# Sorax5/RaytracingEngine

Hardware: AMD Instinct MI355X
Metric: Mrays/sec (primary+shadow) at 1920x1080 (higher is better)
Workload: dtype f64

## Files before the change

include/rt_capi.h:

```cpp
#ifndef RT_CAPI_H
#define RT_CAPI_H

#include <stddef.h>
#include <stdint.h>

#ifdef __cplusplus
extern "C" {
#endif

#define RT_CAPI_VERSION 1

typedef enum rt_status {
    RT_OK = 0,
    RT_ERR_INVALID_ARG = 1,
    RT_ERR_HIP = 2,
    RT_ERR_OOM = 3,
    RT_ERR_UNSUPPORTED = 4,
    RT_ERR_NO_DEVICE = 5,
    RT_ERR_RCCL = 6
} rt_status;

typedef struct rt_material {
    double color[3];
    double shininess;
// ... 265 lines not shown
#define RT_SC_REFRACT  0x02
#define RT_SC_REFLECT  0x04
#define RT_SC_WEIGHTS  0x08
#define RT_SC_FLAGS    0x10
#define RT_SC_ALL      0x1f
struct rt_scatter_out {
    void* value;
    void* refract_rays;
    void* reflect_rays;
    void* weights;
    void* flags;
};
rt_status rt_scatter_rays(rt_context* ctx, const rt_scene* scene, const rt_render_opts* opts,
                          const double* rays, size_t n, int outputs,
                          const struct rt_scatter_out* out);
rt_status rt_scatter_rays_device(rt_context* ctx, const rt_scene* scene,
                                 const rt_render_opts* opts, const void* d_rays, size_t n,
                                 int outputs, const struct rt_scatter_out* d_out);

rt_status rt_camera_rays(rt_context* ctx, const rt_camera* cam, const rt_render_opts* opts,
                         int sample, double* rays_out);
rt_status rt_camera_rays_device(rt_context* ctx, const rt_camera* cam, const rt_render_opts* opts,
                                int sample, void* d_rays);

#define RT_CH_T        0x01
#define RT_CH_PRIM     0x02
#define RT_CH_NORMAL   0x04
#define RT_CH_POINT    0x08
#define RT_CH_MATERIAL 0x10
#define RT_CH_ALL      0x1f
struct rt_closest_out {
    void* t;
    void* prim;
    void* normal;
    void* point;
    void* material;
};
rt_status rt_closest_rays(rt_context* ctx, const rt_scene* scene, const rt_render_opts* opts,
                          const double* rays, size_t n, int outputs,
                          const struct rt_closest_out* out);
rt_status rt_closest_rays_device(rt_context* ctx, const rt_scene* scene,
                                 const rt_render_opts* opts, const void* d_rays, size_t n,
                                 int outputs, const struct rt_closest_out* d_out);

rt_status rt_trace_rays_device(rt_context* ctx, const rt_scene* scene, const rt_render_opts* opts,
                               const void* d_rays, size_t n, void* d_rgb);

rt_status rt_accumulate_samples_device(rt_context* ctx, const rt_scene* scene,
                                       const rt_camera* cam, const rt_render_opts* opts,
                                       int sample_begin, int sample_end, void* d_sum);
rt_status rt_accumulate_samples(rt_context* ctx, const rt_scene* scene, const rt_camera* cam,
                                const rt_render_opts* opts, int sample_begin, int sample_end,
                                double* sum);

rt_status rt_resolve_device(rt_context* ctx, const void* d_sum, size_t n_pixels, int samples,
                            int tonemap, void* d_hdr64, void* d_hdr32, void* d_ldr);
rt_status rt_resolve(rt_context* ctx, const double* sum, size_t n_pixels, int samples, int tonemap,
                     double* hdr64, float* hdr32, uint8_t* ldr);

rt_status rt_tonemap(rt_context* ctx, const double* hdr, size_t n_pixels, int op,
                     uint8_t* ldr_out);

rt_status rt_debug_f64_ops(rt_context* ctx, const double* x, const double* y, size_t n,
                           double* out);

rt_status rt_debug_vec_ops(rt_context* ctx, const double* v, size_t n, double* out);

rt_status rt_debug_assemble_rows(rt_context* ctx, const void* gathered, size_t row_bytes,
                                 uint32_t height, uint32_t block, uint32_t n, uint32_t max_rows,
                                 void* image);

rt_status rt_debug_tile_order(rt_context* ctx, const rt_scene* scene, const rt_camera* cam,
                              uint32_t* order, uint32_t* cost, size_t capacity, uint32_t* tiles,
                              uint32_t* waves, int* state);

rt_status rt_debug_cone_table(rt_context* ctx, uint64_t* with_table, uint64_t* without_table);

rt_status rt_debug_shadow_table(rt_context* ctx, uint64_t* with_table, uint64_t* without_table);

rt_status rt_debug_tile_class(rt_context* ctx, uint64_t* with_words, uint64_t* without_words);

rt_status rt_debug_plane_clear(rt_context* ctx, uint64_t* with_masks, uint64_t* without_masks);

#ifdef __cplusplus
}
#endif

#endif
```

raytracingengine_amd/capi.py:

```python
from __future__ import annotations

import ctypes
import os

import numpy as np

from .scene import AREA_LIGHT_DTYPE, SceneData

HERE = os.path.dirname(os.path.abspath(__file__))
LIB_PATH = os.environ.get("RTAMD_LIB", os.path.join(HERE, "librtamd.so"))

(RT_OK, RT_ERR_INVALID_ARG, RT_ERR_HIP, RT_ERR_OOM, RT_ERR_UNSUPPORTED, RT_ERR_NO_DEVICE,
 RT_ERR_RCCL) = range(7)
STATUS_NAMES = {0: "RT_OK", 1: "RT_ERR_INVALID_ARG", 2: "RT_ERR_HIP", 3: "RT_ERR_OOM",
                4: "RT_ERR_UNSUPPORTED", 5: "RT_ERR_NO_DEVICE", 6: "RT_ERR_RCCL"}

TONEMAP_NONE = -1
TONEMAPS = ["simple", "reinhard_simple", "reinhard_extended", "reinhard_extended_luminance",
            "reinhard_jodie", "uncharted2", "aces"]
TONEMAP_ALL = 7
RT_FLAG_COUNT_RAYS = 0x1
RT_FLAG_TIME_KERNEL = 0x2
RT_FLAG_GENERIC_KERNEL = 0x4
RT_FLAG_NO_BVH = 0x8
RT_FLAG_PIPELINE = 0x10
RT_FLAG_NO_TILE_ORDER = 0x20
RT_FLAG_NO_SAMPLE_PARALLEL = 0x40
RT_OUT_HDR64, RT_OUT_HDR32, RT_OUT_LDR = 0x1, 0x2, 0x4
RT_COMM_ID_BYTES = 128
GB_DEPTH = 0x01
GB_DEPTH_NORM = 0x02
GB_NORMAL = 0x04
GB_PRIM = 0x08
GB_ALBEDO = 0x10
GB_ALL = 0x1F
DL_RADIANCE = 0x1
DL_DIFFUSE = 0x2
DL_SPECULAR = 0x4
DL_ALL = 0x7
DL_OUTPUTS = [("radiance", DL_RADIANCE), ("diffuse", DL_DIFFUSE), ("specular", DL_SPECULAR)]
SC_VALUE = 0x01
SC_REFRACT = 0x02
SC_REFLECT = 0x04
SC_WEIGHTS = 0x08
SC_FLAGS = 0x10
SC_ALL = 0x1F
SC_OUTPUTS = [("value", SC_VALUE, np.float64, 3), ("refract_rays", SC_REFRACT, np.float64, 6),
              ("reflect_rays", SC_REFLECT, np.float64, 6), ("weights", SC_WEIGHTS, np.float64, 2),
              ("flags", SC_FLAGS, np.uint8, 0)]
CH_T = 0x01
CH_PRIM = 0x02
CH_NORMAL = 0x04
CH_POINT = 0x08
CH_MATERIAL = 0x10
CH_ALL = 0x1F
CH_OUTPUTS = [("t", CH_T, np.float64, 0), ("prim", CH_PRIM, np.int32, 2),
              ("normal", CH_NORMAL, np.float64, 3), ("point", CH_POINT, np.float64, 3),
              ("material", CH_MATERIAL, np.float64, 7)]
GB_OUTPUTS = [("depth", GB_DEPTH, np.float64, 1), ("depth_norm", GB_DEPTH_NORM, np.float32, 1),
              ("normal", GB_NORMAL, np.float64, 3), ("prim", GB_PRIM, np.int32, 2),
              ("albedo", GB_ALBEDO, np.float32, 3)]

EXPORTED = [
    "rt_last_error", "rt_build_info", "rt_device_count", "rt_render_opts_default", "rt_context_create",
    "rt_context_destroy", "rt_context_set_stream", "rt_context_synchronize", "rt_scene_create",
    "rt_scene_destroy", "rt_scene_set_area_light", "rt_render", "rt_render_device",
    "rt_render_multi", "rt_comm_unique_id", "rt_comm_create", "rt_comm_create_all",
    "rt_comm_create_local", "rt_comm_destroy", "rt_comm_info", "rt_comm_set_root_weight",
    "rt_comm_create_ex", "rt_comm_set_timeout", "rt_render_gather", "rt_render_gather_all",
    "rt_comm_timing", "rt_comm_synchronize", "rt_debug_assemble_rows", "rt_debug_tile_order",
    "rt_stats_read", "rt_stats_reset", "rt_trace_rays", "rt_intersect_rays", "rt_tonemap",
    "rt_debug_f64_ops", "rt_debug_vec_ops", "rt_queue_create", "rt_queue_destroy",
    "rt_queue_submit", "rt_queue_wait", "rt_queue_synchronize", "rt_render_batch",
    "rt_render_gather_batch", "rt_render_gather_all_batch", "rt_gbuffer", "rt_gbuffer_device",
    "rt_debug_cone_table",
    "rt_debug_shadow_table",
    "rt_debug_tile_class",
    "rt_debug_plane_clear",
    "rt_occluded_rays", "rt_occluded_rays_device",
    "rt_transmittance_rays", "rt_transmittance_rays_device",
    "rt_light_transmittance", "rt_light_transmittance_device",
    "rt_direct_light", "rt_direct_light_device",
    "rt_direct_light_rays", "rt_direct_light_rays_device",
    "rt_scatter_rays", "rt_scatter_rays_device",
    "rt_camera_rays", "rt_camera_rays_device",
    "rt_closest_rays", "rt_closest_rays_device",
    "rt_trace_rays_device",
    "rt_accumulate_samples", "rt_accumulate_samples_device",
    "rt_resolve", "rt_resolve_device",
]


class RtError(RuntimeError):
    def __init__(self, status: int, msg: str):
        super().__init__(f"{STATUS_NAMES.get(status, status)}: {msg}")
        self.status = status


class SceneDesc(ctypes.Structure):
    _fields_ = [
        ("spheres", ctypes.c_void_p), ("n_spheres", ctypes.c_int32),
        ("planes", ctypes.c_void_p), ("n_planes", ctypes.c_int32),
        ("triangles", ctypes.c_void_p), ("n_triangles", ctypes.c_int32),
        ("lights", ctypes.c_void_p), ("n_lights", ctypes.c_int32),
    ]


class RenderOpts(ctypes.Structure):
    _fields_ = [
        ("max_recursion", ctypes.c_int32), ("tonemap", ctypes.c_int32),
        ("bias", ctypes.c_double), ("seed", ctypes.c_uint64),
        ("row_begin", ctypes.c_uint32), ("row_end", ctypes.c_uint32),
        ("flags", ctypes.c_int32), ("row_block", ctypes.c_uint16), ("row_cycle", ctypes.c_uint16),
    ]


class Stats(ctypes.Structure):
    _fields_ = [
        ("trace_rays", ctypes.c_uint64), ("shadow_rays", ctypes.c_uint64),
        ("kernel_ms", ctypes.c_double), ("launches", ctypes.c_uint64),
    ]


class GBufferPtrs(ctypes.Structure):
    _fields_ = [(name, ctypes.c_void_p) for name, _, _, _ in GB_OUTPUTS]


def gbuffer_layout(outputs: int, width: int, rows: int, frames: int | None = None) -> dict:
    if outputs == 0 or outputs & ~GB_ALL:
        raise ValueError(f"G-buffer outputs {outputs:#x}: no output or an unknown bit")
    lead = () if frames is None else (int(frames),)
    return {name: (lead + (rows, width) + ((k,) if k > 1 else ()), np.dtype(dt))
            for name, bit, dt, k in GB_OUTPUTS if outputs & bit}


class DirectLightPtrs(ctypes.Structure):
    _fields_ = [(name, ctypes.c_void_p) for name, _ in DL_OUTPUTS]


def material_rows(materials, n: int) -> np.ndarray:
    if hasattr(materials, "as_tuple"):
        c, *rest = materials.as_tuple()
        materials = (*c, *rest)
    m = np.ascontiguousarray(materials, np.float64)
    if m.ndim == 1:
        m = m.reshape(1, -1)
    if m.ndim != 2 or m.shape[1] != 7 or m.shape[0] not in (1, n):
        raise ValueError("materials: a Material, seven values, or an [n, 7] array")
    return m


class ScatterPtrs(ctypes.Structure):
    _fields_ = [(name, ctypes.c_void_p) for name, *_ in SC_OUTPUTS]


def _sc_check(outputs: int):
    if outputs == 0 or outputs & ~SC_ALL:
        raise ValueError("outputs: a non-empty combination of SC_* bits")


class ClosestPtrs(ctypes.Structure):
# ... 29 lines not shown
        import torch
    except ImportError:
        pass
    if not os.path.exists(path):
        raise RuntimeError(
            f"{path} is missing: build it with `python -c 'import __graft_entry__ as g; g.build()'`"
            " (hipcc --offload-arch=gfx950). The renderer has no CPU fallback.")
    L = ctypes.CDLL(path)
    vp, i32 = ctypes.c_void_p, ctypes.c_int
    L.rt_last_error.restype = ctypes.c_char_p
    if hasattr(L, "rt_build_info") or "RTAMD_LIB" not in os.environ:
        L.rt_build_info.restype = ctypes.c_char_p
        L.rt_build_info.argtypes = []
    L.rt_device_count.restype = i32
    L.rt_render_opts_default.argtypes = [vp]
    L.rt_render_opts_default.restype = None
    for name, args in {
        "rt_context_create": [i32, vp],
        "rt_context_destroy": [vp],
        "rt_context_set_stream": [vp, vp],
        "rt_context_synchronize": [vp],
        "rt_scene_create": [vp, vp, vp],
        "rt_scene_destroy": [vp],
        "rt_scene_set_area_light": [vp, vp],
        "rt_render": [vp, vp, vp, vp, vp, vp, vp, vp],
        "rt_render_device": [vp, vp, vp, vp, vp, vp, vp],
        "rt_render_batch": [vp, vp, vp, i32, vp, vp, vp, vp],
        "rt_gbuffer": [vp, vp, vp, vp, i32, vp],
        "rt_gbuffer_device": [vp, vp, vp, i32, vp, i32, vp],
        "rt_render_multi": [vp, vp, i32, vp, vp, vp, vp, vp, vp],
        "rt_stats_read": [vp, vp],
        "rt_stats_reset": [vp],
        "rt_trace_rays": [vp, vp, vp, vp, ctypes.c_size_t, vp, vp],
        "rt_intersect_rays": [vp, vp, vp, ctypes.c_size_t, vp],
        "rt_occluded_rays": [vp, vp, vp, vp, vp, ctypes.c_size_t, vp],
        "rt_occluded_rays_device": [vp, vp, vp, vp, vp, ctypes.c_size_t, vp],
        "rt_transmittance_rays": [vp, vp, vp, vp, vp, ctypes.c_size_t, vp],
        "rt_transmittance_rays_device": [vp, vp, vp, vp, vp, ctypes.c_size_t, vp],
        "rt_light_transmittance": [vp, vp, vp, vp, ctypes.c_size_t, vp],
        "rt_light_transmittance_device": [vp, vp, vp, vp, ctypes.c_size_t, vp],
        "rt_direct_light": [vp, vp, vp, vp, vp, ctypes.c_size_t, ctypes.c_size_t, i32, vp],
        "rt_direct_light_device": [vp, vp, vp, vp, vp, ctypes.c_size_t, ctypes.c_size_t, i32, vp],
        "rt_direct_light_rays": [vp, vp, vp, vp, ctypes.c_size_t, i32, vp],
        "rt_direct_light_rays_device": [vp, vp, vp, vp, ctypes.c_size_t, i32, vp],
        "rt_scatter_rays": [vp, vp, vp, vp, ctypes.c_size_t, i32, vp],
        "rt_scatter_rays_device": [vp, vp, vp, vp, ctypes.c_size_t, i32, vp],
        "rt_camera_rays": [vp, vp, vp, i32, vp],
        "rt_camera_rays_device": [vp, vp, vp, i32, vp],
        "rt_closest_rays": [vp, vp, vp, vp, ctypes.c_size_t, i32, vp],
        "rt_closest_rays_device": [vp, vp, vp, vp, ctypes.c_size_t, i32, vp],
        "rt_trace_rays_device": [vp, vp, vp, vp, ctypes.c_size_t, vp],
        "rt_accumulate_samples": [vp, vp, vp, vp, i32, i32, vp],
        "rt_accumulate_samples_device": [vp, vp, vp, vp, i32, i32, vp],
        "rt_resolve": [vp, vp, ctypes.c_size_t, i32, i32, vp, vp, vp],
        "rt_resolve_device": [vp, vp, ctypes.c_size_t, i32, i32, vp, vp, vp],
        "rt_tonemap": [vp, vp, ctypes.c_size_t, i32, vp],
        "rt_debug_f64_ops": [vp, vp, vp, ctypes.c_size_t, vp],
        "rt_debug_vec_ops": [vp, vp, ctypes.c_size_t, vp],
        "rt_comm_unique_id": [vp],
        "rt_comm_create": [vp, i32, i32, vp, vp],
        "rt_comm_create_ex": [vp, i32, i32, vp, ctypes.c_long, vp],
        "rt_comm_set_timeout": [vp, ctypes.c_long],
        "rt_comm_create_all": [vp, i32, vp],
        "rt_comm_create_local": [vp, i32, vp],
        "rt_comm_destroy": [vp],
        "rt_comm_info": [vp, vp, vp],
        "rt_comm_set_root_weight": [vp, i32],
        "rt_render_gather": [vp, vp, vp, vp, i32, vp, vp, vp],
        "rt_render_gather_all": [vp, vp, i32, vp, vp, i32, vp, vp, vp],
        "rt_render_gather_batch": [vp, vp, vp, i32, vp, i32, vp, vp, vp, vp, vp, vp],
        "rt_render_gather_all_batch": [vp, vp, i32, vp, i32, vp, i32, vp, vp, vp],
        "rt_comm_timing": [vp, vp, i32],
        "rt_comm_synchronize": [vp],
        "rt_queue_create": [vp, i32, vp],
        "rt_queue_destroy": [vp],
        "rt_queue_submit": [vp, vp, vp, vp, vp, vp, vp, vp],
        "rt_queue_wait": [vp, ctypes.c_uint64],
        "rt_queue_synchronize": [vp],
        "rt_debug_tile_order": [vp, vp, vp, vp, vp, ctypes.c_size_t, vp, vp, vp],
        "rt_debug_cone_table": [vp, vp, vp],
        "rt_debug_shadow_table": [vp, vp, vp],
        "rt_debug_tile_class": [vp, vp, vp],
        "rt_debug_plane_clear": [vp, vp, vp],
        "rt_debug_assemble_rows": [vp, vp, ctypes.c_size_t, ctypes.c_uint32, ctypes.c_uint32,
                                   ctypes.c_uint32, ctypes.c_uint32, vp],
    }.items():
        try:
            fn = getattr(L, name)
        except AttributeError:
            if "RTAMD_LIB" in os.environ:
                continue
            raise
        fn.argtypes = args
        fn.restype = i32
    _lib = L
    return L


def build_info() -> dict:
    import json
    info = json.loads(load_library().rt_build_info().decode())
    from . import build
    info["matches_tree"] = info.get("source_sha256") == build.source_digest()
    return info


def _check(status: int):
    if status != RT_OK:
        raise RtError(status, _lib.rt_last_error().decode(errors="replace"))


def rendered_rows(o: RenderOpts, height: int) -> int:
    r1 = min(o.row_end, height) if o.row_end else height
    if r1 <= o.row_begin:
        return 0
    if o.row_cycle <= 1 or o.row_block == 0:
        return r1 - o.row_begin
    stride = o.row_block * o.row_cycle
    return sum(min(o.row_block, r1 - b) for b in range(o.row_begin, r1, stride))


def default_opts(**kw) -> RenderOpts:
    o = RenderOpts()
    load_library().rt_render_opts_default(ctypes.byref(o))
    for k, v in kw.items():
        setattr(o, k, v)
    return o


def device_count() -> int:
    return load_library().rt_device_count()


def progressive_schedule(aa_samples: int) -> list:
    n = max(1, int(aa_samples))
    steps, k = [], 1
    while k < n:
        steps.append(k)
        k *= 2
    return steps + [n]


class Context:

    def __init__(self, device: int = 0):
        L = load_library()
        self._h = ctypes.c_void_p()
        _check(L.rt_context_create(device, ctypes.byref(self._h)))
        self.device = device

    def close(self):
        if self._h:
            _lib.rt_context_destroy(self._h)
            self._h = ctypes.c_void_p()

    def __del__(self):
        try:
            self.close()
        except Exception:
            pass

    def __enter__(self):
        return self

    def __exit__(self, *exc):
        self.close()

    @property
    def handle(self):
        return self._h

    def set_stream(self, stream_ptr: int | None):
        _check(_lib.rt_context_set_stream(self._h, stream_ptr))

    def synchronize(self):
        _check(_lib.rt_context_synchronize(self._h))

    def scene(self, sc: SceneData) -> "DeviceScene":
        return DeviceScene(self, sc)

    def stats(self) -> Stats:
        s = Stats()
        _check(_lib.rt_stats_read(self._h, ctypes.byref(s)))
        return s

    def reset_stats(self):
        _check(_lib.rt_stats_reset(self._h))

    def tonemap(self, hdr: np.ndarray, op: int) -> np.ndarray:
        hdr = np.ascontiguousarray(hdr, np.float64).reshape(-1, 3)
        planes = 7 if op == TONEMAP_ALL else 1
        out = np.empty((planes, hdr.shape[0], 3), np.uint8)
        _check(_lib.rt_tonemap(self._h, hdr.ctypes.data, hdr.shape[0], op, out.ctypes.data))
        return out if planes > 1 else out[0]

    def debug_f64_ops(self, x: np.ndarray, y: np.ndarray) -> np.ndarray:
        x = np.ascontiguousarray(x, np.float64)
        y = np.ascontiguousarray(y, np.float64)
        out = np.empty((x.size, 5), np.float64)
        _check(_lib.rt_debug_f64_ops(self._h, x.ctypes.data, y.ctypes.data, x.size,
                                     out.ctypes.data))
        return out

    def debug_assemble_rows(self, gathered: np.ndarray, height: int, block: int, n: int,
                            max_rows: int) -> np.ndarray:
        g = np.ascontiguousarray(gathered, np.uint8).reshape(n, max_rows, -1)
        out = np.empty((height, g.shape[2]), np.uint8)
        _check(_lib.rt_debug_assemble_rows(self._h, g.ctypes.data, g.shape[2], height, block, n,
                                           max_rows, out.ctypes.data))
        return out

    def debug_cone_table(self) -> tuple[int, int]:
        a, b = ctypes.c_uint64(), ctypes.c_uint64()
        _check(_lib.rt_debug_cone_table(self._h, ctypes.byref(a), ctypes.byref(b)))
        return a.value, b.value

    def debug_shadow_table(self) -> tuple[int, int]:
        a, b = ctypes.c_uint64(), ctypes.c_uint64()
        _check(_lib.rt_debug_shadow_table(self._h, ctypes.byref(a), ctypes.byref(b)))
        return a.value, b.value

    def debug_tile_class(self) -> tuple[int, int]:
        a, b = ctypes.c_uint64(), ctypes.c_uint64()
        _check(_lib.rt_debug_tile_class(self._h, ctypes.byref(a), ctypes.byref(b)))
        return a.value, b.value

    def debug_plane_clear(self) -> tuple[int, int]:
        a, b = ctypes.c_uint64(), ctypes.c_uint64()
        _check(_lib.rt_debug_plane_clear(self._h, ctypes.byref(a), ctypes.byref(b)))
        return a.value, b.value

    def debug_vec_ops(self, v: np.ndarray) -> np.ndarray:
        v = np.ascontiguousarray(v, np.float64).reshape(-1, 3)
        out = np.empty((v.shape[0], 16), np.float64)
        _check(_lib.rt_debug_vec_ops(self._h, v.ctypes.data, v.shape[0], out.ctypes.data))
        return out


class DeviceScene:

    def __init__(self, ctx: Context, sc: SceneData):
        self.ctx = ctx
        self.data = sc
        self._arrays = (sc.sphere_array(), sc.plane_array(), sc.triangle_array(), sc.light_array())
        sp, pl, tr, lt = self._arrays
        desc = SceneDesc(sp.ctypes.data if len(sp) else None, len(sp),
                         pl.ctypes.data if len(pl) else None, len(pl),
                         tr.ctypes.data if len(tr) else None, len(tr),
                         lt.ctypes.data if len(lt) else None, len(lt))
        self._h = ctypes.c_void_p()
        _check(_lib.rt_scene_create(ctx.handle, ctypes.byref(desc), ctypes.byref(self._h)))
        self.camera = sc.camera.to_struct()
        self._area = None
        if sc.area_light is not None:
            self._area = sc.area_light.to_struct()
            _check(_lib.rt_scene_set_area_light(self._h, self._area.ctypes.data))

    def close(self):
        if self._h:
            _lib.rt_scene_destroy(self._h)
            self._h = ctypes.c_void_p()

    def __del__(self):
        try:
            self.close()
        except Exception:
            pass

    def render(self, *, hdr64=True, hdr32=False, tonemap: int = TONEMAP_NONE, opts=None,
               stats=False, **opt_kw):
        cam = self.data.camera
        o = opts if opts is not None else default_opts(tonemap=tonemap, **opt_kw)
        if opts is None:
            o.tonemap = tonemap
        rows = rendered_rows(o, cam.height)
        out = {}
        a64 = np.empty((rows, cam.width, 3), np.float64) if hdr64 else None
        a32 = np.empty((rows, cam.width, 3), np.float32) if hdr32 else None
        ldr = np.empty((rows, cam.width, 3), np.uint8) if tonemap != TONEMAP_NONE else None
        st = Stats()
        _check(_lib.rt_render(self.ctx.handle, self._h, self.camera.ctypes.data, ctypes.byref(o),
                              a64.ctypes.data if a64 is not None else None,
                              a32.ctypes.data if a32 is not None else None,
                              ldr.ctypes.data if ldr is not None else None,
                              ctypes.byref(st) if stats else None))
        if a64 is not None:
            out["hdr64"] = a64
        if a32 is not None:
            out["hdr32"] = a32
        if ldr is not None:
            out["ldr"] = ldr
        if stats:
            out["trace_rays"] = st.trace_rays
            out["shadow_rays"] = st.shadow_rays
        return out

    def render_host(self, h_hdr64: int | None, h_hdr32: int | None, h_ldr: int | None,
                    opts: RenderOpts, stats: bool = False):
        st = Stats()
        _check(_lib.rt_render(self.ctx.handle, self._h, self.camera.ctypes.data, ctypes.byref(opts),
                              h_hdr64, h_hdr32, h_ldr, ctypes.byref(st) if stats else None))
        return st if stats else None

    def trace_rays(self, rays: np.ndarray, stats=False, **opt_kw):
        rays = np.ascontiguousarray(rays, np.float64).reshape(-1, 6)
        out = np.empty((rays.shape[0], 3), np.float64)
        o = default_opts(**opt_kw)
        st = Stats()
        _check(_lib.rt_trace_rays(self.ctx.handle, self._h, ctypes.byref(o), rays.ctypes.data,
                                  rays.shape[0], out.ctypes.data,
                                  ctypes.byref(st) if stats else None))
        return (out, st) if stats else out
# ... 702 lines not shown
```

raytracingengine_amd/csrc/rt_capi.cpp:

```cpp
#include "rt_capi.h"

#include <hip/hip_runtime.h>

#include <algorithm>
#include <cmath>
#include <cstdlib>
#include <cstdio>
#include <cstring>
#include <mutex>
#include <new>
#include <string>
#include <utility>
#include <vector>

#include "rt_context.hpp"
#include "rt_internal.hpp"
#include "rt_wavefront.hpp"

#pragma clang fp contract(off)

using namespace rtamd;

namespace rtamd {

// ... 202 lines not shown
        if (ctx->scratch_used) RT_HIP(hipEventSynchronize(ctx->scratch_event));
        RT_HIP(ctx->fix_list.ensure(px * sizeof(uint32_t)));
    }
    p.fix_list = static_cast<uint32_t*>(ctx->fix_list.ptr);
    p.fix_ctl = static_cast<uint32_t*>(ctx->fix_ctl.ptr) + ctx->fix_parity;
    p.fix_next = static_cast<uint32_t*>(ctx->fix_ctl.ptr) + (1 - ctx->fix_parity);
    return RT_OK;
}

rt_status check_batch(const rt_camera* cams, int nframes) {
    if (!cams || nframes < 1) return fail(RT_ERR_INVALID_ARG, "frame batch: no cameras");
    for (int f = 0; f < nframes; ++f) {
        rt_status st = validate_camera(cams + f);
        if (st != RT_OK) return st;
        if (cams[f].width != cams[0].width || cams[f].height != cams[0].height ||
            cams[f].aa_samples != cams[0].aa_samples ||
            std::memcmp(&cams[f].focal, &cams[0].focal, sizeof(double)) != 0)
            return fail(RT_ERR_INVALID_ARG, "frame batch: every camera must have the first's "
                                            "width, height, focal and aa_samples");
    }
    return RT_OK;
}

rt_status enqueue_render(rt_context* ctx, const rt_scene* sc, const rt_camera* cam,
                         const rt_render_opts* opts, double* d64, float* d32, uint8_t* dldr) {
    return enqueue_frames(ctx, sc, cam, 1, opts, d64, d32, dldr);
}

rt_status enqueue_frames(rt_context* ctx, const rt_scene* sc, const rt_camera* cams, int nframes,
                         const rt_render_opts* opts, double* d64, float* d32, uint8_t* dldr,
                         uint32_t frame_rows) {
    TraceParams p;
    int path;
    bool lds;
    size_t lds_bytes;
    uint32_t rows;
    rt_status st = nframes == 1 ? RT_OK : check_batch(cams, nframes);
    if (st != RT_OK) return st;
    st = build_params(ctx, sc, cams, opts, p, path, lds, lds_bytes, rows);
    if (st != RT_OK) return st;
    p.out64 = d64;
    p.out32 = d32;
    p.ldr = dldr;
    const int flags = opts ? opts->flags : 0;
    if (!dldr) p.tonemap = RT_TONEMAP_NONE;
    if (dldr && p.tonemap == RT_TONEMAP_NONE) p.ldr = nullptr;
    const bool packet_path = path == kPathDirect && !(flags & RT_FLAG_GENERIC_KERNEL) &&
                             p.ns <= packet_max_spheres() &&
                             packet_lds_bytes(p.ns, p.np, p.nl) <= ctx->lds_limit;
    if (frame_rows && frame_rows < rows)
        return fail(RT_ERR_INVALID_ARG, "frame batch: frame stride below the rendered rows");
    const size_t frame_px = static_cast<size_t>(frame_rows ? frame_rows : rows) * p.width;
    if (nframes > 1 && (!packet_path || nframes > kPkMaxBatch)) {
        const int step = packet_path ? kPkMaxBatch : 1;
        for (int f0 = 0; f0 < nframes; f0 += step) {
            const size_t off = 3 * frame_px * static_cast<size_t>(f0);
            st = enqueue_frames(ctx, sc, cams + f0, std::min(step, nframes - f0), opts,
                                d64 ? d64 + off : nullptr, d32 ? d32 + off : nullptr,
                                dldr ? dldr + off : nullptr, frame_rows);
            if (st != RT_OK) return st;
        }
        return RT_OK;
    }
    bool scratch = (flags & RT_FLAG_COUNT_RAYS) || uses_wavefront_arena(path, flags);

    std::pair<hipEvent_t, hipEvent_t> ev{nullptr, nullptr};
    if (flags & RT_FLAG_TIME_KERNEL) {
        if (ctx->pending.size() >= 1024) {
            st = harvest_events(ctx, false);
            if (st != RT_OK) return st;
        }
        if (!ctx->free_events.empty()) {
            ev = ctx->free_events.back();
            ctx->free_events.pop_back();
        } else {
            RT_HIP(hipEventCreate(&ev.first));
            RT_HIP(hipEventCreate(&ev.second));
        }
        RT_HIP(hipEventRecord(ev.first, ctx->stream));
    }
    const bool packet = packet_path;
    rt_scene::PkImage::TileOrder* rec = nullptr;
    int batch_ring = -1;
    if (packet && nframes > 1) {
        p.nframes = static_cast<uint32_t>(nframes);
        p.frame_px = frame_px;
        st = packet_batch_images(ctx, sc, cams, nframes, p, flags, &rec, &batch_ring);
        if (st != RT_OK) return st;
    } else if (packet) {
        st = packet_image(ctx, sc, p, flags, &rec);
        if (st != RT_OK) return st;
    }
    if (packet) {
        for (int f = 0; f < nframes; ++f)
            ++((nframes > 1 ? p.fr_tab[f] : p.cone_tab) ? ctx->cone_tab_frames
                                                         : ctx->cone_notab_frames);
        for (int f = 0; f < nframes; ++f)
            ++((nframes > 1 ? p.fr_stab[f] : p.shadow_tab) ? ctx->shadow_tab_frames
                                                            : ctx->shadow_notab_frames);
        for (int f = 0; f < nframes; ++f)
            ++((nframes > 1 ? p.fr_ctab[f] : p.class_tab) ? ctx->tile_class_frames
                                                          : ctx->tile_noclass_frames);
        for (int f = 0; f < nframes; ++f)
            ++(((nframes > 1 ? p.fr_ctab[f] : p.class_tab) && p.plane_masks)
                   ? ctx->plane_mask_frames
                   : ctx->plane_nomask_frames);
    }
    const bool fixup = packet && packet_uses_fixup(p, false, sc->max_specular > 0.0);
    if (fixup) {
        st = fixup_buffers(ctx, nframes > 1 ? static_cast<size_t>(nframes) * frame_px
                                             : static_cast<size_t>(rows) * p.width, p);
        if (st != RT_OK) return st;
        scratch = true;
    }
    if (scratch) {
        st = scratch_wait(ctx);
        if (st != RT_OK) return st;
    }
    const bool lean_generic = p.nt == 0 && p.al_samples == 0;
    static const bool box_sph = [] {
        const char* e = std::getenv("RTAMD_BOX_SPH");
        return !(e && std::atoi(e) == 0);
    }();
    const bool box = path == kPathChain && p.nt == 0 && p.al_samples == 0 &&
                     (p.ns == 0 ? p.np > 0 : (box_sph && p.ns <= kBoxMaxSpheres)) &&
                     !(flags & RT_FLAG_GENERIC_KERNEL);
    const bool spar = !(flags & RT_FLAG_NO_SAMPLE_PARALLEL);
    auto launch = [&](const TraceParams& q, bool count) {
        if (box)
            return launch_box_chain(q, count, !(flags & RT_FLAG_NO_SAMPLE_PARALLEL), ctx->stream);
        return packet ? launch_packet_direct(q, count, sc->max_specular > 0.0, ctx->stream)
                      : (lean_generic ? lean::launch_trace(q, path, count, lds, lds_bytes, ctx->stream, spar)
                                      : launch_trace(q, path, count, lds, lds_bytes, ctx->stream, spar));
    };
    bool wavefront = false;
    if (uses_wavefront_arena(path, flags)) {
        const size_t n0 = static_cast<size_t>(rows) * p.width *
                          static_cast<size_t>(p.aa > 0 ? p.aa : 0);
        const char* env = std::getenv("RTAMD_WF_MB");
        const size_t budget = (env && std::atoll(env) > 0 ? static_cast<size_t>(std::atoll(env))
                                                          : size_t(4096)) << 20;
        const bool defer = path == kPathTree && wf_defer_selected();
        const size_t root_bytes = wf_arena_bytes(n0, n0, defer);
        if (n0 < (size_t(1) << 30) && root_bytes <= budget) {
            size_t extra = (budget - root_bytes) / (defer ? 116 : 100);
            extra = std::min(extra, std::max<size_t>(n0, 1) * 64);
            extra = std::min(extra, (size_t(1) << 31) - 1 - n0);
            const size_t cap = n0 + extra;
            RT_HIP(ctx->wf.ensure(wf_arena_bytes(n0, cap, defer)));
            RT_HIP(ctx->wf_ctl.ensure(sizeof(WfCtl)));
            const WfArena A = wf_arena_layout(ctx->wf.ptr, n0, cap,
                                              static_cast<WfCtl*>(ctx->wf_ctl.ptr), defer);
            RT_HIP(lean_generic ? lean::launch_wavefront(p, path, A, lds, lds_bytes, ctx->stream)
                                : launch_wavefront(p, path, A, lds, lds_bytes, ctx->stream));
            wavefront = true;
        }
    }
    if (!wavefront) RT_HIP(launch(p, false));
    if (fixup) {
        const hipError_t fe = launch_packet_fixup(p, ctx->stream);
        if (fe != hipSuccess) {
            (void)hipMemsetAsync(ctx->fix_ctl.ptr, 0, 2 * sizeof(uint32_t), ctx->stream);
            return hip_fail(fe, "launch_packet_fixup");
        }
        ctx->fix_parity ^= 1;
    }
    if (rec) RT_HIP(hipEventRecord(rec->recorded, ctx->stream));
    if (flags & RT_FLAG_TIME_KERNEL) {
        RT_HIP(hipEventRecord(ev.second, ctx->stream));
        ctx->pending.push_back(ev);
    }
    if (flags & RT_FLAG_COUNT_RAYS) {
        TraceParams pc = p;
        pc.out64 = nullptr;
        pc.out32 = nullptr;
        pc.ldr = nullptr;
        pc.counters = static_cast<unsigned long long*>(ctx->counters.ptr);
        pc.tile_cost = nullptr;
        RT_HIP(launch(pc, true));
    }
    if (batch_ring >= 0) {
        RT_HIP(hipEventRecord(sc->pk_batch_done[batch_ring], ctx->stream));
        sc->pk_batch_used[batch_ring] = true;
    }
    return scratch ? scratch_done(ctx) : RT_OK;
}

constexpr size_t kGbBytes[5] = {8, 4, 24, 8, 12};

rt_status check_gbuffer_args(int outputs, const rt_gbuffer_out* out) {
    if (outputs == 0) return fail(RT_ERR_INVALID_ARG, "G-buffer: no output requested");
    if (outputs & ~RT_GB_ALL) return fail(RT_ERR_INVALID_ARG, "G-buffer: unknown output bit");
    if (!out) return fail(RT_ERR_INVALID_ARG, "G-buffer: the output record is NULL");
    const void* ptr[5] = {out->depth, out->depth_norm, out->normal, out->prim, out->albedo};
    for (int k = 0; k < 5; ++k)
        if ((outputs & (1 << k)) && !ptr[k])
            return fail(RT_ERR_INVALID_ARG, "G-buffer: a requested output's pointer is NULL");
    return RT_OK;
}

rt_status enqueue_gbuffer(rt_context* ctx, const rt_scene* sc, const rt_camera* cams, int nframes,
                          const rt_render_opts* opts_in, int outputs, const rt_gbuffer_out& out) {
    rt_status st = check_batch(cams, nframes);
    if (st != RT_OK) return st;
    rt_render_opts opts;
    if (opts_in) opts = *opts_in;
    else rt_render_opts_default(&opts);
    opts.max_recursion = 1;
    opts.tonemap = RT_TONEMAP_NONE;
    opts.flags &= RT_FLAG_GENERIC_KERNEL | RT_FLAG_NO_BVH | RT_FLAG_TIME_KERNEL;
    TraceParams p;
    int path;
    bool lds;
    size_t lds_bytes;
// ... 242 lines not shown
    }

    if (sc->ns >= kSphChunkMin) {
        std::vector<int32_t> perm;
        std::vector<double> bnd;
        build_sphere_chunks(&h[sc->off_sph], sc->ns, perm, bnd);
        sc->off_sbnd = (h.size() + 1) & ~size_t(1);
        sc->off_sperm = sc->off_sbnd + bnd.size();
        h.resize(sc->off_sperm + (perm.size() + 1) / 2 + 2, 0.0);
        std::memcpy(&h[sc->off_sbnd], bnd.data(), bnd.size() * sizeof(double));
        std::memcpy(&h[sc->off_sperm], perm.data(), perm.size() * sizeof(int32_t));
    }

    if (sc->np > 0) {
        std::vector<int> grp(sc->np);
        for (int i = 0; i < sc->np; ++i) {
            const double* q = &h[sc->off_pl + size_t(kPlStride) * i];
            const double* n = q + 3;
            grp[i] = 3;
            const bool bounded = std::fabs(q[0]) <= 0x1p1000 && std::fabs(q[1]) <= 0x1p1000 &&
                                 std::fabs(q[2]) <= 0x1p1000;
            for (int k = 0; k < 3 && bounded; ++k)
                if (std::fabs(n[k]) == 1.0 && n[(k + 1) % 3] == 0.0 && n[(k + 2) % 3] == 0.0)
                    grp[i] = k;
        }
        sc->off_box = (h.size() + 1) & ~size_t(1);
        h.resize(sc->off_box + size_t(kBoxRec) * sc->np + 2, 0.0);
        size_t r = 0;
        for (int g = 0; g < 4; ++g) {
            for (int i = 0; i < sc->np; ++i) {
                if (grp[i] != g) continue;
                const double* pl = &h[sc->off_pl + size_t(kPlStride) * i];
                double* o = &h[sc->off_box + size_t(kBoxRec) * r++];
                for (int k = 0; k < 6; ++k) o[k] = pl[k];
                o[6] = g < 3 ? pl[g] : 0.0;
                const double nn = pl[3] * pl[3] + pl[4] * pl[4] + pl[5] * pl[5];
                o[7] = std::sqrt(nn) == 1.0 ? 1.0 : 0.0;
                for (int k = 0; k < kMatStride - 1; ++k)
                    o[8 + k] = h[sc->off_pl_mat + size_t(kMatStride) * i + k];
                const int32_t idx[2] = {i, 0};
                std::memcpy(&o[15], idx, sizeof idx);
                ++sc->box_n[g];
            }
        }
    }

    hipError_t e = sc->buf.ensure(h.size() * sizeof(double));
    if (e == hipSuccess)
        e = hipMemcpyAsync(sc->buf.ptr, h.data(), h.size() * sizeof(double),
                           hipMemcpyHostToDevice, ctx->stream);
    if (e == hipSuccess) e = hipStreamSynchronize(ctx->stream);
    if (e != hipSuccess) {
        sc->buf.release();
        delete sc;
        return hip_fail(e, "rt_scene_create upload");
    }
    *out = sc;
    return RT_OK;
}

rt_status rt_scene_destroy(rt_scene* sc) {
    if (!sc) return RT_OK;
    DeviceGuard g(sc->ctx->device);
    (void)hipDeviceSynchronize();
    sc->buf.release();
    sc->pk_pub.release();
    sc->pk_batch.release();
    for (auto& e : sc->pk_batch_done)
        if (e) (void)hipEventDestroy(e);
    for (auto& im : sc->pk_images) {
        im.buf.release();
        if (im.ready) (void)hipEventDestroy(im.ready);
        for (auto& o : im.ords) {
            o.cost.release();
            o.keys.release();
            o.order.release();
            if (o.recorded) (void)hipEventDestroy(o.recorded);
            if (o.built) (void)hipEventDestroy(o.built);
            if (o.verdict) (void)hipHostFree(o.verdict);
        }
        for (auto& t : im.tabs) {
            t.buf.release();
            if (t.ready) (void)hipEventDestroy(t.ready);
        }
    }
    for (auto& b : sc->pk_batch_tab) b.release();
    delete sc;
    return RT_OK;
}

rt_status rt_scene_set_area_light(rt_scene* sc, const rt_area_light* light) {
    if (!sc) return fail(RT_ERR_INVALID_ARG, "scene is NULL");
    if (!light) {
        sc->has_area = false;
        return RT_OK;
    }
    if (light->samples <= 0) return fail(RT_ERR_INVALID_ARG, "area light needs samples > 0");
    const int k = static_cast<int>(std::lround(std::sqrt(static_cast<double>(light->samples))));
    if (k * k != light->samples)
        return fail(RT_ERR_INVALID_ARG, "area light samples must be a perfect square");
    sc->area = *light;
    sc->has_area = true;
    return RT_OK;
}

rt_status rt_render_device(rt_context* ctx, const rt_scene* sc, const rt_camera* cam,
                           const rt_render_opts* opts, void* d64, void* d32, void* dldr) {
    if (!ctx) return fail(RT_ERR_INVALID_ARG, "context is NULL");
    DeviceGuard g(ctx->device);
    return enqueue_render(ctx, sc, cam, opts, static_cast<double*>(d64), static_cast<float*>(d32),
                   static_cast<uint8_t*>(dldr));
}

rt_status rt_render_batch(rt_context* ctx, const rt_scene* sc, const rt_camera* cams,
                          int nframes, const rt_render_opts* opts, void* d64, void* d32,
                          void* dldr) {
    if (!ctx) return fail(RT_ERR_INVALID_ARG, "context is NULL");
    rt_status st = check_batch(cams, nframes);
    if (st != RT_OK) return st;
    DeviceGuard g(ctx->device);
    return enqueue_frames(ctx, sc, cams, nframes, opts, static_cast<double*>(d64),
                          static_cast<float*>(d32), static_cast<uint8_t*>(dldr));
}

rt_status rt_gbuffer_device(rt_context* ctx, const rt_scene* sc, const rt_camera* cams,
                            int nframes, const rt_render_opts* opts, int outputs,
                            const struct rt_gbuffer* d_out) {
    rt_status st = check_gbuffer_args(outputs, d_out);
    if (st != RT_OK) return st;
    if (!ctx) return fail(RT_ERR_INVALID_ARG, "context is NULL");
    DeviceGuard g(ctx->device);
    return enqueue_gbuffer(ctx, sc, cams, nframes, opts, outputs, *d_out);
}

rt_status rt_gbuffer(rt_context* ctx, const rt_scene* sc, const rt_camera* cam,
                     const rt_render_opts* opts, int outputs, const struct rt_gbuffer* h_out) {
    rt_status st = check_gbuffer_args(outputs, h_out);
    if (st != RT_OK) return st;
    if (!ctx) return fail(RT_ERR_INVALID_ARG, "context is NULL");
    st = validate_camera(cam);
    if (st != RT_OK) return st;
    DeviceGuard g(ctx->device);
    rt_render_opts o;
    if (opts) o = *opts;
    else rt_render_opts_default(&o);
    const size_t npx = static_cast<size_t>(rendered_rows(o, cam->height)) * cam->width;
    void* const host[5] = {h_out->depth, h_out->depth_norm, h_out->normal, h_out->prim,
                           h_out->albedo};
    size_t off[5], total = 0;
    for (int k = 0; k < 5; ++k) {
        off[k] = total;
        if (outputs & (1 << k)) total += (npx * kGbBytes[k] + 255) / 256 * 256;
    }
    RT_HIP(ctx->out64.ensure(total));
    char* base = static_cast<char*>(ctx->out64.ptr);
    rt_gbuffer_out d{base + off[0], base + off[1], base + off[2], base + off[3], base + off[4]};
    st = enqueue_gbuffer(ctx, sc, cam, 1, &o, outputs, d);
    if (st != RT_OK) return st;
    for (int k = 0; k < 5; ++k)
        if (outputs & (1 << k))
            RT_HIP(hipMemcpyAsync(host[k], base + off[k], npx * kGbBytes[k], hipMemcpyDeviceToHost,
                                  ctx->stream));
    RT_HIP(hipStreamSynchronize(ctx->stream));
    return RT_OK;
}

// ... 863 lines not shown
    return RT_OK;
}

rt_status rt_debug_f64_ops(rt_context* ctx, const double* x, const double* y, size_t n,
                           double* out) {
    if (!ctx || !x || !y || !out) return fail(RT_ERR_INVALID_ARG, "NULL argument");
    DeviceGuard g(ctx->device);
    RT_HIP(ctx->dbg.ensure(n * 7 * sizeof(double)));
    double* dx = static_cast<double*>(ctx->dbg.ptr);
    double* dy = dx + n;
    double* dout = dy + n;
    RT_HIP(hipMemcpyAsync(dx, x, n * sizeof(double), hipMemcpyHostToDevice, ctx->stream));
    RT_HIP(hipMemcpyAsync(dy, y, n * sizeof(double), hipMemcpyHostToDevice, ctx->stream));
    RT_HIP(launch_debug_f64(dx, dy, n, dout, ctx->stream));
    RT_HIP(hipMemcpyAsync(out, dout, 5 * n * sizeof(double), hipMemcpyDeviceToHost, ctx->stream));
    RT_HIP(hipStreamSynchronize(ctx->stream));
    return RT_OK;
}

rt_status rt_debug_tile_order(rt_context* ctx, const rt_scene* sc, const rt_camera* cam,
                              uint32_t* order, uint32_t* cost, size_t capacity, uint32_t* tiles,
                              uint32_t* waves, int* state) {
    if (!ctx || !sc || !cam || !tiles || !waves || !state)
        return fail(RT_ERR_INVALID_ARG, "NULL argument to rt_debug_tile_order");
    *tiles = *waves = 0;
    *state = 0;
    DeviceGuard g(ctx->device);
    RT_HIP(hipDeviceSynchronize());
    for (const auto& im : sc->pk_images) {
        if (std::memcmp(im.cam, cam->position, sizeof im.cam) != 0) continue;
        if (im.last_ord < 0) return RT_OK;
        const auto& o = im.ords[static_cast<size_t>(im.last_ord)];
        *state = o.state;
        if (o.state == 0) return RT_OK;
        *tiles = o.key[0] * o.key[1];
        *waves = o.key[2];
        if (order && o.state == 2) {
            if (capacity < *tiles) return fail(RT_ERR_INVALID_ARG, "order capacity too small");
            RT_HIP(hipMemcpy(order, o.order.ptr, sizeof(uint32_t) * *tiles, hipMemcpyDeviceToHost));
        }
        if (cost) {
            if (capacity < size_t(*tiles) * *waves)
                return fail(RT_ERR_INVALID_ARG, "cost capacity too small");
            RT_HIP(hipMemcpy(cost, o.cost.ptr, sizeof(uint32_t) * *tiles * *waves,
                             hipMemcpyDeviceToHost));
        }
        return RT_OK;
    }
    return RT_OK;
}

rt_status rt_debug_cone_table(rt_context* ctx, uint64_t* with_table, uint64_t* without_table) {
    if (!ctx || !with_table || !without_table)
        return fail(RT_ERR_INVALID_ARG, "NULL argument to rt_debug_cone_table");
    *with_table = ctx->cone_tab_frames;
    *without_table = ctx->cone_notab_frames;
    return RT_OK;
}

rt_status rt_debug_shadow_table(rt_context* ctx, uint64_t* with_table, uint64_t* without_table) {
    if (!ctx || !with_table || !without_table)
        return fail(RT_ERR_INVALID_ARG, "NULL argument to rt_debug_shadow_table");
    *with_table = ctx->shadow_tab_frames;
    *without_table = ctx->shadow_notab_frames;
    return RT_OK;
}

rt_status rt_debug_tile_class(rt_context* ctx, uint64_t* with_words, uint64_t* without_words) {
    if (!ctx || !with_words || !without_words)
        return fail(RT_ERR_INVALID_ARG, "NULL argument to rt_debug_tile_class");
    *with_words = ctx->tile_class_frames;
    *without_words = ctx->tile_noclass_frames;
    return RT_OK;
}

rt_status rt_debug_plane_clear(rt_context* ctx, uint64_t* with_masks, uint64_t* without_masks) {
    if (!ctx || !with_masks || !without_masks)
        return fail(RT_ERR_INVALID_ARG, "NULL argument to rt_debug_plane_clear");
    *with_masks = ctx->plane_mask_frames;
    *without_masks = ctx->plane_nomask_frames;
    return RT_OK;
}

rt_status rt_debug_vec_ops(rt_context* ctx, const double* v, size_t n, double* out) {
    if (!ctx || !v || !out) return fail(RT_ERR_INVALID_ARG, "NULL argument");
    DeviceGuard g(ctx->device);
    RT_HIP(ctx->dbg.ensure(n * 19 * sizeof(double)));
    double* dv = static_cast<double*>(ctx->dbg.ptr);
    double* dout = dv + 3 * n;
    RT_HIP(hipMemcpyAsync(dv, v, 3 * n * sizeof(double), hipMemcpyHostToDevice, ctx->stream));
    RT_HIP(launch_debug_vec(dv, n, dout, ctx->stream));
    RT_HIP(hipMemcpyAsync(out, dout, 16 * n * sizeof(double), hipMemcpyDeviceToHost, ctx->stream));
    RT_HIP(hipStreamSynchronize(ctx->stream));
    return RT_OK;
}

}
```

raytracingengine_amd/csrc/rt_context.hpp:

```cpp
#pragma once

#include <hip/hip_runtime.h>

#include <array>
#include <string>
#include <utility>
#include <vector>

#include "rt_capi.h"
#include "rt_internal.hpp"

namespace rtamd {

rt_status fail(rt_status st, const std::string& msg);
rt_status hip_fail(hipError_t e, const char* what);

#define RT_HIP(call)                                    \
    do {                                                \
        hipError_t e_ = (call);                         \
        if (e_ != hipSuccess) return rtamd::hip_fail(e_, #call); \
    } while (0)

struct DeviceBuffer {
    void* ptr = nullptr;
    size_t bytes = 0;
    hipError_t ensure(size_t need) {
        if (need <= bytes) return hipSuccess;
        if (ptr) (void)hipFree(ptr);
        ptr = nullptr;
        bytes = 0;
        hipError_t e = hipMalloc(&ptr, need);
        if (e == hipSuccess) bytes = need;
        return e;
    }
    void release() {
        if (ptr) (void)hipFree(ptr);
        ptr = nullptr;
        bytes = 0;
    }
};

struct DeviceGuard {
    int prev = -1;
    explicit DeviceGuard(int dev) {
        if (hipGetDevice(&prev) != hipSuccess) prev = -1;
        (void)hipSetDevice(dev);
    }
    ~DeviceGuard() {
        if (prev >= 0) (void)hipSetDevice(prev);
    }
};

}

struct rt_comm;

struct rt_context {
    int device = 0;
    hipStream_t stream = nullptr;
    hipStream_t own_stream = nullptr;
    size_t lds_limit = 0;
    rtamd::DeviceBuffer out64, out32, ldr, tm_in, tm_out, dbg, rays;
    rtamd::DeviceBuffer counters;
    rtamd::DeviceBuffer wf, wf_ctl;
    hipEvent_t scratch_event = nullptr;
    bool scratch_used = false;
    hipStream_t scratch_stream = nullptr;
    rtamd::DeviceBuffer fix_list, fix_ctl;
    int fix_parity = 0;
    std::vector<std::pair<hipEvent_t, hipEvent_t>> pending;
    std::vector<std::pair<hipEvent_t, hipEvent_t>> free_events;
    double timed_ms = 0.0;
    uint64_t launches = 0;
    uint64_t cone_tab_frames = 0, cone_notab_frames = 0;
    uint64_t shadow_tab_frames = 0, shadow_notab_frames = 0;
    uint64_t tile_class_frames = 0, tile_noclass_frames = 0;
    uint64_t plane_mask_frames = 0, plane_nomask_frames = 0;
    std::vector<rt_context*> group_ctxs;
    std::vector<rt_comm*> group_comms;
    std::vector<rt_context*> group_roots;
};

struct rt_scene {
    rt_context* ctx = nullptr;
    rtamd::DeviceBuffer buf;
    int32_t ns = 0, np = 0, nt = 0, nl = 0;
    size_t off_sph = 0, off_sph_mat = 0, off_pl = 0, off_pl_mat = 0, off_tri = 0, off_tri_mat = 0,
           off_lt = 0;
    bool any_transparent = false;
    double max_specular = 0.0;
    bool has_area = false;
    rt_area_light area{};
    size_t off_bvh = 0, off_bvh_tri = 0;
    int32_t bvh_nodes = 0;
    size_t off_sperm = 0, off_sbnd = 0;
    size_t off_box = 0;
    int32_t box_n[4] = {0, 0, 0, 0};
    struct PkImage {
        double cam[3];
        rtamd::DeviceBuffer buf;
        hipEvent_t ready = nullptr;
        hipStream_t stream = nullptr;
        bool done = false;
        struct TileOrder {
            uint32_t key[8] = {};
            int state = 0;
            rtamd::DeviceBuffer cost, keys, order;
            hipEvent_t recorded = nullptr, built = nullptr;
            uint32_t* verdict = nullptr;
        };
        std::vector<TileOrder> ords;
        int last_ord = -1;
        struct ConeTab {
            static constexpr size_t kKeyWords = 20;
            uint32_t key[kKeyWords] = {};
            rtamd::DeviceBuffer buf;
            hipEvent_t ready = nullptr;
            hipStream_t stream = nullptr;
            bool done = false;
        };
        std::vector<ConeTab> tabs;
    };
    mutable std::vector<PkImage> pk_images;
    mutable std::vector<std::array<double, 3>> pk_seen;
    mutable rtamd::DeviceBuffer pk_pub;
    static constexpr int kPkBatchRing = 4;
    mutable rtamd::DeviceBuffer pk_batch;
    mutable hipEvent_t pk_batch_done[kPkBatchRing] = {nullptr, nullptr, nullptr, nullptr};
    mutable bool pk_batch_used[kPkBatchRing] = {false, false, false, false};
    mutable int pk_batch_next = 0;
    mutable rtamd::DeviceBuffer pk_batch_tab[kPkBatchRing];
};

namespace rtamd {

uint32_t rendered_rows(const rt_render_opts& o, uint32_t height);
rt_status validate_camera(const rt_camera* cam);
rt_status enqueue_render(rt_context* ctx, const rt_scene* sc, const rt_camera* cam,
                         const rt_render_opts* opts, double* d64, float* d32, uint8_t* dldr);
rt_status enqueue_frames(rt_context* ctx, const rt_scene* sc, const rt_camera* cams, int nframes,
                         const rt_render_opts* opts, double* d64, float* d32, uint8_t* dldr,
                         uint32_t frame_rows = 0);
rt_status check_batch(const rt_camera* cams, int nframes);
rt_status packet_image(rt_context* ctx, const rt_scene* sc, TraceParams& p, int flags,
                       rt_scene::PkImage::TileOrder** rec);
rt_status packet_batch_images(rt_context* ctx, const rt_scene* sc, const rt_camera* cams,
                              int nframes, TraceParams& p, int flags,
                              rt_scene::PkImage::TileOrder** rec, int* batch_ring);
bool uses_wavefront_arena(int path, int flags);
rt_status scratch_wait(rt_context* ctx);
rt_status scratch_done(rt_context* ctx);
rt_status harvest_events(rt_context* ctx, bool all);
void release_group(rt_context* ctx);
void leave_groups(rt_context* ctx);

}
```

raytracingengine_amd/csrc/rt_internal.hpp:

```cpp
#pragma once

#include <hip/hip_runtime.h>
#include <stddef.h>
#include <stdint.h>

#include <vector>

namespace rtamd {

constexpr int kSphStride = 4;
constexpr int kPlStride = 8;
constexpr int kTriStride = 12;
constexpr int kLtStride = 8;
constexpr int kMatStride = 8;
constexpr int kBoxRec = 16;
constexpr int kBoxMaxSpheres = 64;

constexpr int kBvhNodeStride = 8;
constexpr int kBvhMinTris = 32;
constexpr int kBvhStack = 64;
constexpr int kMaxDepth = 16;
constexpr int kTileW = 8;
constexpr int kTileH = 32;

enum PathKind : int {
    kPathDirect = 0,
    kPathChain = 1,
    kPathTree = 2
};

constexpr int kPkMaxBatch = 32;
struct PkFrame {
    double cam[3];
    const double* img;
    unsigned long long* pub;
    uint32_t epoch;
    uint32_t _pad;
};

struct TraceParams {
    const double* sph;
    const double* sph_mat;
    const double* pl;
    const double* pl_mat;
    const double* tri;
    const double* tri_mat;
    const double* lt;
    int32_t ns, np, nt, nl;
    double al_corner[3];
    double al_u[3];
    double al_v[3];
    double al_E[3];
    int32_t al_samples;
    int32_t al_k;
    double cam_pos[3];
    double focal;
    uint32_t width, height;
    int32_t aa;
    int32_t max_rec;
    double bias;
    uint64_t seed;
    uint32_t row0, rows;
    uint32_t row_block, row_stride;
    double* out64;
    float* out32;
    uint8_t* ldr;
    int32_t tonemap;
    int32_t _pad;
    unsigned long long* counters;
    const uint8_t* redo;
    const double* bvh;
    const int32_t* bvh_tri;
    const double* pk_image;
    unsigned long long* pk_pub;
    uint32_t pk_epoch;
    uint32_t pk_pub_first;
    const int32_t* sph_perm;
    const double* sph_bnd;
    const uint32_t* redo_any;
    const uint32_t* tile_order;
    uint32_t* tile_cost;
    const double* box;
    int32_t box_n[4];
    uint32_t* fix_list;
    uint32_t* fix_ctl;
    uint32_t* fix_next;
    uint32_t nframes;
    uint32_t plane_masks;
    uint64_t frame_px;
    PkFrame fr[kPkMaxBatch];
    double half_w, half_h, cam_dz, cam_dz2;
    double fr_dz[kPkMaxBatch][2];
    const unsigned long long* cone_tab;
    const unsigned long long* fr_tab[kPkMaxBatch];
    const unsigned long long* shadow_tab;
    const unsigned long long* fr_stab[kPkMaxBatch];
    const unsigned long long* class_tab;
    const unsigned long long* fr_ctab[kPkMaxBatch];
};
static_assert(sizeof(TraceParams) + 12 * kPkMaxBatch + 32 <= 4096, "kernel arguments above 4 KiB");

struct CameraConsts {
    double half_w, half_h, dz, dz2;
};
inline CameraConsts camera_consts(uint32_t width, uint32_t height, double cam_z, double focal) {
    CameraConsts c;
    c.half_w = static_cast<double>(width) / 2.0;
    c.half_h = static_cast<double>(height) / 2.0;
    c.dz = (cam_z + focal) - cam_z;
    c.dz2 = c.dz * c.dz;
    return c;
}

constexpr int kSphChunkMin = 65;
void build_sphere_chunks(const double* sph, int ns, std::vector<int32_t>& perm,
                         std::vector<double>& bounds);

void build_triangle_bvh(const double* tri, int nt, std::vector<double>& nodes,
                        std::vector<int32_t>& order);

__host__ __device__ inline size_t scene_doubles(const TraceParams& p) {
    return static_cast<size_t>(kSphStride) * p.ns + static_cast<size_t>(kPlStride) * p.np +
           static_cast<size_t>(kLtStride) * p.nl;
}

constexpr int kAaParallelMax = 128;
hipError_t launch_trace(const TraceParams& p, int path, bool count, bool lds, size_t lds_bytes,
                        hipStream_t stream, bool sample_parallel = false);
namespace lean {
hipError_t launch_trace(const TraceParams& p, int path, bool count, bool lds, size_t lds_bytes,
                        hipStream_t stream, bool sample_parallel = false);
}
hipError_t launch_box_chain(const TraceParams& p, bool count, bool sample_parallel,
                            hipStream_t stream);
hipError_t launch_packet_direct(const TraceParams& p, bool count, bool any_specular,
                                hipStream_t stream);
size_t packet_lds_bytes(int ns, int np, int nl);
hipError_t launch_packet_image(const TraceParams& p, double* img, hipStream_t stream);
bool packet_uses_fixup(const TraceParams& p, bool count, bool any_specular);
hipError_t launch_packet_fixup(const TraceParams& p, hipStream_t stream);
struct PkImageJobs {
    double* dst[kPkMaxBatch];
    int32_t frame[kPkMaxBatch];
    int32_t n;
};
hipError_t launch_packet_image_batch(const TraceParams& p, const PkImageJobs& jobs,
                                     hipStream_t stream);
struct PkConeJobs {
    unsigned long long* dst[kPkMaxBatch];
    int32_t frame[kPkMaxBatch];
    int32_t n;
    int32_t shadow_nl;
    int32_t class_words;
};
hipError_t launch_packet_cone_tables(const TraceParams& p, const PkConeJobs& jobs,
                                     hipStream_t stream);
bool packet_reads_cone_table(const TraceParams& p, bool any_specular);
int packet_shadow_table_lights(const TraceParams& p);
void packet_grid(const TraceParams& p, uint32_t& gx, uint32_t& gy, uint32_t& waves);
hipError_t launch_packet_order(const uint32_t* cost, uint32_t gx, uint32_t gy, uint32_t waves,
                               uint32_t* keys, uint32_t* order, uint32_t* verdict,
                               hipStream_t stream);
int packet_max_spheres();
struct GbOut {
    double* depth;
    float* depth_norm;
    double* normal;
    int32_t* prim;
    float* albedo;
    double planes[kPkMaxBatch][2];
};
bool gbuffer_packet_fits(const TraceParams& p, size_t lds_limit);
hipError_t launch_gbuffer(const TraceParams& p, const GbOut& g, bool packet, int tile_w,
                          hipStream_t stream);
hipError_t launch_trace_rays(const TraceParams& p, int path, bool count, const double* rays,
                             size_t n, double* out, hipStream_t stream);
hipError_t launch_intersect_rays(const TraceParams& p, const double* rays, size_t n, double* out,
                                 hipStream_t stream);
hipError_t launch_occluded_rays(const TraceParams& p, const double* rays, const double* max_dist,
                                size_t n, uint8_t* out, hipStream_t stream);
hipError_t launch_transmittance_rays(const TraceParams& p, bool opaque, const double* rays,
                                     const double* max_dist, size_t n, double* out,
                                     hipStream_t stream);
hipError_t launch_light_transmittance(const TraceParams& p, bool opaque, const double* points,
                                      size_t n, double* out, hipStream_t stream);
struct DlOut {
    double* radiance;
    double* diffuse;
    double* specular;
};
struct DlMaterial {
    double v[8];
};
hipError_t launch_direct_light_points(const TraceParams& p, bool opaque, const double* points,
                                      const double* materials, const DlMaterial& shared, size_t n,
                                      const DlOut& out, hipStream_t stream);
hipError_t launch_direct_light_rays(const TraceParams& p, bool opaque, const double* rays, size_t n,
                                    const DlOut& out, hipStream_t stream);
struct ScOut {
    double* value;
    double* refract_rays;
    double* reflect_rays;
    double* weights;
    uint8_t* flags;
};
hipError_t launch_scatter_rays(const TraceParams& p, bool opaque, const double* rays, size_t n,
                               const ScOut& out, hipStream_t stream);
hipError_t launch_camera_rays(const TraceParams& p, int sample, double* out, hipStream_t stream);
struct ChOut {
    double* t;
    int32_t* prim;
    double* normal;
    double* point;
    double* material;
};
hipError_t launch_closest_rays(const TraceParams& p, const double* rays, size_t n, const ChOut& out,
                               hipStream_t stream);
hipError_t launch_accumulate_samples(const TraceParams& p, int path, int s0, int s1, double* sum,
                                     hipStream_t stream);
hipError_t launch_resolve(const double* sum, size_t n, int samples, int op, double* out64,
                          float* out32, uint8_t* ldr, hipStream_t stream);
hipError_t launch_tonemap(const double* hdr, size_t n, int op, uint8_t* out, hipStream_t stream);
hipError_t launch_debug_f64(const double* x, const double* y, size_t n, double* out,
                            hipStream_t stream);
hipError_t launch_debug_vec(const double* v, size_t n, double* out, hipStream_t stream);

}
```

raytracingengine_amd/csrc/rt_packet.hip:

```cpp
#include "rt_cone_table.hpp"
#include "rt_packet_kernel.hpp"
#include "rt_shadow_table.hpp"

#pragma clang fp contract(off)

namespace rtamd {

#ifdef RT_PACKET_PROBE
template __global__ void packet_direct_kernel<RT_PACKET_PROBE>(TraceParams);
#else
size_t packet_lds_bytes(int ns, int np, int nl) { return pk_image_bytes(ns, np, nl); }

__global__ __launch_bounds__(256) void packet_image_kernel(TraceParams P, double* img) {
    pk_build_image(P, P.cam_pos, img, static_cast<int>(threadIdx.x), 256);
}

hipError_t launch_packet_image(const TraceParams& p, double* img, hipStream_t stream) {
    hipLaunchKernelGGL(packet_image_kernel, dim3(1), dim3(256), 0, stream, p, img);
    return hipGetLastError();
}

__global__ __launch_bounds__(256) void packet_image_batch_kernel(TraceParams P, PkImageJobs J) {
    const int f = J.frame[blockIdx.x];
    pk_build_image(P, P.fr[f].cam, J.dst[blockIdx.x], static_cast<int>(threadIdx.x), 256);
}

hipError_t launch_packet_image_batch(const TraceParams& p, const PkImageJobs& jobs,
                                     hipStream_t stream) {
    if (jobs.n <= 0) return hipSuccess;
    if (jobs.n > kPkMaxBatch) return hipErrorInvalidValue;
    for (int j = 0; j < jobs.n; ++j)
        if (!jobs.dst[j] || jobs.frame[j] < 0 || jobs.frame[j] >= static_cast<int>(p.nframes))
            return hipErrorInvalidValue;
    hipLaunchKernelGGL(packet_image_batch_kernel, dim3(static_cast<unsigned>(jobs.n)),
                       dim3(256), 0, stream, p, jobs);
    return hipGetLastError();
}

constexpr int kConeThreads = 256;
__global__ __launch_bounds__(kConeThreads, 5) void packet_cone_table_kernel(TraceParams P,
                                                                         PkConeJobs J, uint32_t gx,
                                                                         uint32_t gy,
                                                                         uint32_t waves) {
    __shared__ float s_terms[64 * 8];
    __shared__ double s_ctr[64 * 3];
    const int f = J.frame[blockIdx.y];
    const double* camp = f < 0 ? P.cam_pos : P.fr[f].cam;
    const double* img = f < 0 ? P.pk_image : P.fr[f].img;
    const double dz = f < 0 ? P.cam_dz : P.fr_dz[f][0];
    const int ns = P.ns < 64 ? P.ns : 64;
    for (int i = threadIdx.x; i < 8 * ns; i += kConeThreads)
        s_terms[i] = reinterpret_cast<const float*>(img + kPkSph * (i >> 3) + 4)[i & 7];
    if (J.shadow_nl > 0)
        for (int i = threadIdx.x; i < 3 * ns; i += kConeThreads)
            s_ctr[i] = img[kPkSph * (i / 3) + i % 3];
    __syncthreads();
    const uint32_t t = blockIdx.x * kConeThreads + threadIdx.x;
    if (t >= gx * gy * waves) return;
    const uint32_t wave = t % waves, wg = t / waves, tbx = wg % gx, tby = wg / gx;
    const uint32_t x0 = tbx * (kPkW * kWgWavesX) + (wave % kWgWavesX) * kPkW;
    const uint32_t yl0 = tby * (kPkH * (waves / kWgWavesX)) + (wave / kWgWavesX) * kPkH;
    const ConeRowPlan rp{P.row0, P.rows, P.row_block, P.row_stride};
    const ConeRect q = cone_tile_rect(x0, yl0, P.width, rp);
    const ConeBound B = cone_tile_bound(q, P.half_w, P.half_h, camp[0], camp[1], dz);
    const uint64_t cone = cone_tile_mask(B, s_terms, 8, ns);
    J.dst[blockIdx.y][t] = cone;
    if (J.shadow_nl <= 0) return;
    unsigned long long* sw = J.dst[blockIdx.y] + static_cast<size_t>(gx) * gy * waves +
                             static_cast<size_t>(t) * J.shadow_nl;
    ShadowBound<2> SB;
    SB.n = 0;
    SB.ok = false;
    if (cone == 0)
        SB = shadow_tile_bound<2>(q, P.half_w, P.half_h, camp, dz, img + kPkSph * ns, P.np, P.bias);
    unsigned long long any = 0, keep = 0;
    for (int l = 0; l < J.shadow_nl; ++l) {
        sw[l] = shadow_tile_word(SB, P.lt + kLtStride * l, P.bias, s_ctr, 3, s_terms + 7, 8, ns);
        any |= sw[l];
        const unsigned k = J.class_words == 2
                               ? shadow_plane_keep<2>(SB, P.lt + kLtStride * l, img + kPkSph * ns,
                                                      P.np, camp, P.bias)
                               : kPlaneKeepAll;
        keep |= static_cast<unsigned long long>(k) << (8 + 8 * l);
    }
    if (J.class_words == 0) return;
    const double* pln = img + kPkSph * ns + kPlStride * P.np + kLtStride * P.nl;
    J.dst[blockIdx.y][static_cast<size_t>(gx) * gy * waves * (1 + J.shadow_nl) + t] =
        tile_class_word(cone, SB, &any, 1, pln, P.np) | keep;
}

hipError_t launch_packet_cone_tables(const TraceParams& p, const PkConeJobs& jobs,
                                     hipStream_t stream) {
    if (jobs.n <= 0) return hipSuccess;
    if (jobs.n > kPkMaxBatch || p.ns > 64 || p.width == 0 || p.rows == 0)
        return hipErrorInvalidValue;
    if (jobs.shadow_nl != 0 && jobs.shadow_nl != packet_shadow_table_lights(p))
        return hipErrorInvalidValue;
    if (jobs.class_words != 0 && jobs.shadow_nl <= 0) return hipErrorInvalidValue;
    if (jobs.class_words < 0 || jobs.class_words > 2) return hipErrorInvalidValue;
    for (int j = 0; j < jobs.n; ++j) {
        const int f = jobs.frame[j];
        if (!jobs.dst[j] || f < -1 || f >= static_cast<int>(p.nframes) ||
            !(f < 0 ? p.pk_image : p.fr[f].img))
            return hipErrorInvalidValue;
    }
    uint32_t gx, gy, waves;
    packet_grid(p, gx, gy, waves);
    const uint32_t tiles = gx * gy * waves;
    hipLaunchKernelGGL(packet_cone_table_kernel,
                       dim3((tiles + kConeThreads - 1) / kConeThreads,
                            static_cast<unsigned>(jobs.n)),
                       dim3(kConeThreads), 0, stream, p, jobs, gx, gy, waves);
    return hipGetLastError();
}

constexpr int kFixThreads = 256;
constexpr int kFixBlocks = 256;
template <bool LDS>
__global__ __launch_bounds__(kFixThreads) void packet_fixup_kernel(TraceParams P) {
    extern __shared__ double smem[];
    const uint32_t n = *P.fix_ctl;
    if (blockIdx.x == 0 && threadIdx.x == 0) *P.fix_next = 0u;
    if (blockIdx.x * kFixThreads >= n) return;
    SceneView S = stage_scene<LDS>(P, smem, threadIdx.x, kFixThreads);
    S.nt = 0;
    S.al = 0;
    S.spec = false;
    S.tri = S.tri_mat = S.bvh = nullptr;
    S.bvh_tri = nullptr;
    Counts cnt{0u, 0u};
    const uint32_t fpx = P.nframes ? static_cast<uint32_t>(P.frame_px) : 0u;
    for (uint32_t i = blockIdx.x * kFixThreads + threadIdx.x; i < n; i += gridDim.x * kFixThreads) {
        const uint32_t o = P.fix_list[i];
        const uint32_t z = fpx ? o / fpx : 0u;
        const uint32_t pl = o - z * fpx;
        const uint32_t yl = pl / P.width;
        const uint32_t x = pl - yl * P.width;
        const double* cp = P.nframes ? P.fr[z].cam : P.cam_pos;
        const d3 cam = mk(cp[0], cp[1], cp[2]);
        const uint32_t y = image_row(P, yl);
        const uint64_t pix = static_cast<uint64_t>(y) * P.width + x;
        const d3 d = camera_dir(P, cam, x, y, pix, 0);
        d3 acc = mk(0.0, 0.0, 0.0);
        acc = acc + trace_direct<false>(S, P, cam, d, pix, 0u, cnt);
        store_pixel(P, static_cast<size_t>(o), acc);
    }
}

hipError_t launch_packet_fixup(const TraceParams& p, hipStream_t stream) {
    if (!p.fix_list || !p.fix_ctl || !p.fix_next) return hipErrorInvalidValue;
    if (p.nt != 0 || p.al_samples != 0) return hipErrorInvalidValue;
    const size_t lds = sizeof(double) * scene_doubles(p);
    if (lds <= 32 * 1024)
        hipLaunchKernelGGL(packet_fixup_kernel<true>, dim3(kFixBlocks), dim3(kFixThreads), lds,
                           stream, p);
    else
        hipLaunchKernelGGL(packet_fixup_kernel<false>, dim3(kFixBlocks), dim3(kFixThreads), 0,
                           stream, p);
    return hipGetLastError();
}

int packet_max_spheres() { return 16 * 64; }

void packet_grid(const TraceParams& p, uint32_t& gx, uint32_t& gy, uint32_t& waves) {
    const size_t lds = pk_image_bytes(p.ns, p.np, p.nl);
    const uint32_t wgy = pk_wgy(lds);
    gx = (p.width + kPkW * kWgWavesX - 1) / (kPkW * kWgWavesX);
    gy = (p.rows + kPkH * wgy - 1) / (kPkH * wgy);
    waves = kWgWavesX * wgy;
}

constexpr int kOrderBins = 16;
__global__ __launch_bounds__(1024) void packet_order_kernel(const uint32_t* cost, uint32_t gx,
                                                            uint32_t gy, uint32_t waves,
                                                            uint32_t* keys, uint32_t* order,
                                                            uint32_t* verdict) {
    __shared__ uint32_t s_max, s_cnt[kOrderBins];
    const uint32_t tid = threadIdx.x, tiles = gx * gy;
    if (tid == 0) s_max = 0;
    if (tid < kOrderBins) s_cnt[tid] = 0;
    __syncthreads();
    uint32_t m = 0;
    for (uint32_t i = tid; i < tiles; i += blockDim.x) {
        uint32_t c = 0;
        for (uint32_t w = 0; w < waves; ++w) c = max(c, cost[i * waves + w]);
        keys[i] = c;
        m = max(m, c);
    }
    atomicMax(&s_max, m);
    __syncthreads();
    const uint64_t top = static_cast<uint64_t>(s_max) + 1;
    for (uint32_t i = tid; i < tiles; i += blockDim.x) {
        const uint64_t bin = static_cast<uint64_t>(keys[i]) * kOrderBins / top;
        const uint32_t key = kOrderBins - 1 - static_cast<uint32_t>(bin);
        keys[i] = key;
// ... 8 lines not shown
        if (2 * acc >= tiles) {
            median_bin = kOrderBins - 1 - b;
            break;
        }
    }
    const bool narrow = median_bin >= kOrderBins / 4;
    if (tid == 0 && verdict) __hip_atomic_store(verdict, narrow ? 1u : 2u, __ATOMIC_RELAXED,
                                                __HIP_MEMORY_SCOPE_SYSTEM);
    uint32_t cur = 0;
    for (int b = 0; b < kOrderBins; ++b)
        if (static_cast<int>(tid) > b) cur += s_cnt[b];
    if (narrow) {
        for (uint32_t lin = tid; lin < tiles; lin += 64) order[lin] = (gy - 1 - lin / gx) * gx + lin % gx;
        return;
    }
    const uint64_t below = (1ull << tid) - 1ull;
    for (uint32_t c0 = 0; c0 < tiles; c0 += 64) {
        const uint32_t lin = c0 + tid;
        const bool ok = lin < tiles;
        uint32_t tile = 0, key = kOrderBins;
        if (ok) {
            tile = (gy - 1 - lin / gx) * gx + lin % gx;
            key = keys[tile];
        }
        for (int b = 0; b < kOrderBins; ++b) {
            const uint64_t mk_ = __ballot(key == static_cast<uint32_t>(b));
            if (!mk_) continue;
            const uint32_t base = __builtin_amdgcn_readlane(cur, b);
            if (key == static_cast<uint32_t>(b))
                order[base + __builtin_popcountll(mk_ & below)] = tile;
            if (static_cast<int>(tid) == b) cur += __builtin_popcountll(mk_);
        }
    }
}

hipError_t launch_packet_order(const uint32_t* cost, uint32_t gx, uint32_t gy, uint32_t waves,
                               uint32_t* keys, uint32_t* order, uint32_t* verdict,
                               hipStream_t stream) {
    hipLaunchKernelGGL(packet_order_kernel, dim3(1), dim3(1024), 0, stream, cost, gx, gy, waves,
                       keys, order, verdict);
    return hipGetLastError();
}

template <int MAXC>
static void launch_packet_maxc(const TraceParams& p, bool count, size_t lds, int feat,
                               hipStream_t stream) {
    if (feat == kFeatFix) launch_packet_variant<1, kFeatFix>(p, count, lds, stream);
    else if (feat == 0) launch_packet_variant<MAXC, 0>(p, count, lds, stream);
    else if (feat == kFeatPlanes) launch_packet_variant<MAXC, kFeatPlanes>(p, count, lds, stream);
    else if (feat == kFeatTris) launch_packet_variant<MAXC, kFeatTris>(p, count, lds, stream);
    else launch_packet_variant<MAXC, kFeatAll>(p, count, lds, stream);
}

static int packet_features(const TraceParams& p, bool any_specular) {
    int feat = 0;
    if (any_specular) feat |= kFeatSpec;
    if (p.al_samples > 0) feat |= kFeatArea;
    if (p.nt > 0) feat |= kFeatTris;
    if (p.ldr && p.tonemap == 4) feat |= kFeatJodie;
    if (p.np >= 3 && feat == 0) feat = kFeatPlanes;
    return feat;
}

bool packet_reads_cone_table(const TraceParams& p, bool any_specular) {
    return p.aa == 1 && !p.tile_cost && p.ns >= 1 && p.ns <= 64 && p.max_rec > 0 &&
           packet_features(p, any_specular) == 0;
}

int packet_shadow_table_lights(const TraceParams& p) {
    return p.np <= 2 ? shadow_table_lights(p.ns, p.np, p.nl, p.al_samples > 0) : 0;
}

constexpr uint64_t kPkFixMinPixels = 32ull << 20;
bool packet_uses_fixup(const TraceParams& p, bool count, bool any_specular) {
    const char* e = std::getenv("RTAMD_PK_FIX");
    const int mode = e ? std::atoi(e) : -1;
    if (mode == 0) return false;
    const bool eligible = !count && p.aa == 1 && !p.tile_cost && p.nframes >= 1 &&
                          (p.ns + 63) / 64 <= 1 && packet_features(p, any_specular) == 0;
    const uint64_t px = static_cast<uint64_t>(p.nframes) * p.rows * p.width;
    return eligible && (mode == 1 || px >= kPkFixMinPixels);
}

hipError_t launch_packet_direct(const TraceParams& p, bool count, bool any_specular,
                                hipStream_t stream) {
    const size_t lds = packet_lds_bytes(p.ns, p.np, p.nl);
    const int chunks = (p.ns + 63) / 64;
    int feat = packet_features(p, any_specular);
    if (packet_uses_fixup(p, count, any_specular)) {
        if (!p.fix_list || !p.fix_ctl || !p.fix_next) return hipErrorInvalidValue;
        feat = kFeatFix;
    }
    if (feat == kFeatArea) return launch_packet_area(p, count, lds, chunks, stream);
    if (chunks <= 1) launch_packet_maxc<1>(p, count, lds, feat, stream);
    else if (chunks <= 4) launch_packet_maxc<4>(p, count, lds, feat, stream);
    else launch_packet_maxc<16>(p, count, lds, feat, stream);
    return hipGetLastError();
}
#endif

}
```

raytracingengine_amd/csrc/rt_packet_device.hpp:

```cpp
#pragma once

#include <cstdlib>

#include "rt_trace_common.hpp"

#pragma clang fp contract(off)

namespace rtamd {

constexpr int kPkW = 8;
constexpr int kPkH = 8;
#ifndef RT_PK_WAVES_X
#define RT_PK_WAVES_X 2
#endif
constexpr int kWgWavesX = RT_PK_WAVES_X;
constexpr size_t kLdsPerCu = 160 * 1024;
constexpr unsigned pk_wgy(size_t lds) { return 10 * lds <= kLdsPerCu ? 1u : 2u; }
constexpr double kCullRel = 1e-4;
constexpr double kFarRatio = 1e5;
constexpr double kNoWin = 1.0 + 0x1.0p-40;
#ifndef RT_SHADOW_SPLIT
#define RT_SHADOW_SPLIT 1
#endif
#ifndef RT_SHADOW_SPLIT_MIN
#define RT_SHADOW_SPLIT_MIN 16
#endif
constexpr bool kShadowSplit = RT_SHADOW_SPLIT != 0;
constexpr int kShadowSplitMin = RT_SHADOW_SPLIT_MIN;

constexpr int kFeatSpec = 1;
constexpr int kFeatArea = 2;
constexpr int kFeatTris = 4;
constexpr int kFeatJodie = 8;
constexpr int kFeatPlanes = 16;
constexpr int kFeatAll = 31;
constexpr int kFeatNoPL = 32;
constexpr int kFeatFix = 128;
#ifndef RT_PACKET_FIX_WAVES
#define RT_PACKET_FIX_WAVES 8
#endif

constexpr int kPkStack = 64;
#ifndef RT_PACKET_SMALL_WAVES
#define RT_PACKET_SMALL_WAVES 6
#endif
#ifndef RT_PACKET_AREA_WAVES
#define RT_PACKET_AREA_WAVES 6
#endif
#ifndef RT_PACKET_LEAN_WAVES
#define RT_PACKET_LEAN_WAVES 4
#endif
#ifndef RT_PACKET_TRIS_WAVES
#define RT_PACKET_TRIS_WAVES 4
#endif
#ifndef RT_PACKET_AA1_WAVES
#define RT_PACKET_AA1_WAVES 5
#endif

__device__ __forceinline__ int cull_lane() {
    int l;
    __asm__ volatile("v_mbcnt_lo_u32_b32 %0, -1, 0\n\tv_mbcnt_hi_u32_b32 %0, -1, %0" : "=v"(l));
    return l;
}


constexpr int kPkSph = 10;

struct PacketScene {
    const double* sph;
    const double* pl;
    const double* lt;
    const double* tri;
    const double* mat;
    const double* bvh;
    const int32_t* bvh_tri;
    const int32_t* orig;
    int ns, np, nt, nl, nb;
    int* wstk;
};

struct PkHit {
    double t;
    int prim;
};

template <int MAXC>
struct Masks {
    uint64_t m[MAXC];
    uint64_t pm;
};

template <int MAXC>
__device__ __forceinline__ Masks<MAXC> all_candidates(int ns) {
    Masks<MAXC> M;
#pragma unroll
    for (int c = 0; c < MAXC; ++c) {
        const int left = ns - 64 * c;
        M.m[c] = left >= 64 ? ~0ull : (left <= 0 ? 0ull : ((1ull << left) - 1ull));
    }
    M.pm = ~0ull;
    return M;
}

constexpr float kF32Slack = 2e-5f;
constexpr float kF32Up = 1.0f + 1e-6f;

__device__ __forceinline__ float f32_up(double v) { return static_cast<float>(v) * kF32Up; }
__device__ __forceinline__ float dot3f(float ax, float ay, float az, float bx, float by, float bz) {
    return ax * bx + ay * by + az * bz;
}
__device__ __forceinline__ float sqrt_f32(float x) { return __builtin_amdgcn_sqrtf(x); }

__device__ __forceinline__ void cone_terms(const double* s, double radius, d3 o, float* out) {
    const float r = f32_up(radius);
    const float vx = static_cast<float>(s[0] - o.x), vy = static_cast<float>(s[1] - o.y),
                vz = static_cast<float>(s[2] - o.z);
    const float dv2 = dot3f(vx, vy, vz, vx, vy, vz);
    const float rr = r * (1.0f + static_cast<float>(kCullRel));
    const float dv = sqrt_f32(dv2);
    const bool always = !(dv > 1.01f * rr) || !(dv <= static_cast<float>(kFarRatio) * r);
    out[0] = vx;
    out[1] = vy;
// ... 468 lines not shown
```

raytracingengine_amd/csrc/rt_packet_host.cpp:

```cpp
#include <hip/hip_runtime.h>

#include <algorithm>
#include <array>
#include <atomic>
#include <cstdlib>
#include <cstring>

#include "rt_context.hpp"
#include "rt_internal.hpp"

#pragma clang fp contract(off)

namespace rtamd {
namespace {

constexpr size_t kMaxPkImages = 16;
constexpr size_t kMaxPkSeen = 16;
constexpr size_t kMaxTileOrders = 8;
constexpr size_t kPkPubSlots = 32;
constexpr size_t kPkPubMaxWords = 1024;
std::atomic<uint32_t> g_pk_epoch{0};
rt_status packet_publish_slot(rt_context* ctx, const rt_scene* sc, TraceParams& p) {
    const size_t words = packet_lds_bytes(p.ns, p.np, p.nl) / 4;
    static const bool off = [] {
        const char* e = std::getenv("RTAMD_PK_PUB");
        return e && std::atoi(e) == 0;
    }();
    if (off || words > kPkPubMaxWords) return RT_OK;
    const size_t slot = kPkPubMaxWords * sizeof(unsigned long long);
    if (!sc->pk_pub.ptr) {
        RT_HIP(sc->pk_pub.ensure(kPkPubSlots * slot));
        RT_HIP(hipMemsetAsync(sc->pk_pub.ptr, 0, kPkPubSlots * slot, ctx->stream));
        RT_HIP(hipStreamSynchronize(ctx->stream));
    }
    uint32_t ep = ++g_pk_epoch;
    if (ep == 0) ep = ++g_pk_epoch;
    p.pk_epoch = ep;
    static const long first_env = [] {
        const char* e = std::getenv("RTAMD_PK_PUB_FIRST");
        return e ? std::atol(e) : -1L;
    }();
    int cus = 0;
    RT_HIP(hipDeviceGetAttribute(&cus, hipDeviceAttributeMultiprocessorCount, ctx->device));
    p.pk_pub_first = first_env >= 0 ? static_cast<uint32_t>(first_env)
                                    : static_cast<uint32_t>(cus > 0 ? cus : 256) * 10u;
    p.pk_pub = reinterpret_cast<unsigned long long*>(static_cast<char*>(sc->pk_pub.ptr) +
                                                     (ep % kPkPubSlots) * slot);
    return RT_OK;
}
rt_status tile_order(rt_context* ctx, rt_scene::PkImage& im, TraceParams& p, int flags,
                     rt_scene::PkImage::TileOrder** rec, bool existing_only = false) {
    *rec = nullptr;
    if (flags & RT_FLAG_NO_TILE_ORDER) return RT_OK;
    uint32_t gx, gy, waves;
    packet_grid(p, gx, gy, waves);
    const uint32_t key[8] = {gx, gy, waves, p.width, p.height, p.rows, p.row0,
                             (p.row_block << 16) ^ p.row_stride};
    const uint32_t tiles = gx * gy;
    size_t idx = 0;
    while (idx < im.ords.size() && std::memcmp(im.ords[idx].key, key, sizeof key) != 0) ++idx;
    if (existing_only && (idx == im.ords.size() || im.ords[idx].state != 2)) return RT_OK;
    if (idx == im.ords.size()) {
        if (im.ords.size() >= kMaxTileOrders) return RT_OK;
        if (im.ords.capacity() < kMaxTileOrders) im.ords.reserve(kMaxTileOrders);
        im.ords.emplace_back();
        auto& o = im.ords.back();
        im.last_ord = static_cast<int>(idx);
        hipError_t e = o.cost.ensure(sizeof(uint32_t) * tiles * waves);
        if (e == hipSuccess) e = hipEventCreateWithFlags(&o.recorded, hipEventDisableTiming);
        if (e != hipSuccess) {
            o.cost.release();
            im.ords.pop_back();
            im.last_ord = -1;
            return hip_fail(e, "tile order");
        }
        std::memcpy(o.key, key, sizeof key);
        o.state = 1;
        p.tile_cost = static_cast<uint32_t*>(o.cost.ptr);
        *rec = &o;
        return RT_OK;
    }
    auto& o = im.ords[idx];
    im.last_ord = static_cast<int>(idx);
    if (o.state == 1) {
        RT_HIP(o.keys.ensure(sizeof(uint32_t) * tiles));
        RT_HIP(o.order.ensure(sizeof(uint32_t) * tiles));
        if (!o.built) RT_HIP(hipEventCreateWithFlags(&o.built, hipEventDisableTiming));
        if (!o.verdict) RT_HIP(hipHostMalloc(reinterpret_cast<void**>(&o.verdict), sizeof(uint32_t)));
        __atomic_store_n(o.verdict, 0u, __ATOMIC_RELAXED);
        RT_HIP(hipStreamWaitEvent(ctx->stream, o.recorded, 0));
        RT_HIP(launch_packet_order(static_cast<const uint32_t*>(o.cost.ptr), gx, gy, waves,
                                   static_cast<uint32_t*>(o.keys.ptr),
                                   static_cast<uint32_t*>(o.order.ptr), o.verdict, ctx->stream));
        RT_HIP(hipEventRecord(o.built, ctx->stream));
        o.state = 2;
    } else {
        if (__atomic_load_n(o.verdict, __ATOMIC_RELAXED) == 1u) return RT_OK;
        RT_HIP(hipStreamWaitEvent(ctx->stream, o.built, 0));
    }
    p.tile_order = static_cast<const uint32_t*>(o.order.ptr);
    return RT_OK;
}

rt_status scene_tile_order(rt_context* ctx, const rt_scene* sc, TraceParams& p, int flags,
                           rt_scene::PkImage::TileOrder** rec) {
    for (auto& im : sc->pk_images) {
        const rt_status st = tile_order(ctx, im, p, flags, rec, true);
        if (st != RT_OK || p.tile_order) return st;
    }
    return RT_OK;
}

rt_status packet_image_cached(rt_context* ctx, const rt_scene* sc, const double* cam,
                              rt_scene::PkImage** out) {
    *out = nullptr;
    for (auto& im : sc->pk_images) {
        if (std::memcmp(im.cam, cam, sizeof im.cam) != 0) continue;
        if (!im.done && im.stream != ctx->stream) {
            const hipError_t q = hipEventQuery(im.ready);
            if (q == hipSuccess) im.done = true;
            else if (q == hipErrorNotReady) RT_HIP(hipStreamWaitEvent(ctx->stream, im.ready, 0));
            else return hip_fail(q, "hipEventQuery");
        }
        *out = &im;
        return RT_OK;
    }
    return RT_OK;
}

bool packet_second_sighting(const rt_scene* sc, const double* cam) {
    auto& seen = sc->pk_seen;
    auto it = std::find_if(seen.begin(), seen.end(), [&](const std::array<double, 3>& c) {
        return std::memcmp(c.data(), cam, 3 * sizeof(double)) == 0;
    });
    if (it == seen.end()) {
        if (seen.size() >= kMaxPkSeen) seen.erase(seen.begin());
        seen.push_back({cam[0], cam[1], cam[2]});
        return false;
    }
    if (sc->pk_images.size() >= kMaxPkImages) return false;
    seen.erase(it);
    return true;
}

rt_status packet_image_entry(rt_context* ctx, const rt_scene* sc, const double* cam,
                             const TraceParams& p, rt_scene::PkImage** out) {
    *out = nullptr;
    if (sc->pk_images.capacity() < kMaxPkImages) sc->pk_images.reserve(kMaxPkImages);
    sc->pk_images.emplace_back();
    rt_scene::PkImage& im = sc->pk_images.back();
    std::memcpy(im.cam, cam, sizeof im.cam);
    im.stream = ctx->stream;
    hipError_t e = im.buf.ensure(packet_lds_bytes(p.ns, p.np, p.nl));
    if (e == hipSuccess) e = hipEventCreateWithFlags(&im.ready, hipEventDisableTiming);
    if (e != hipSuccess) {
        im.buf.release();
        if (im.ready) (void)hipEventDestroy(im.ready);
        sc->pk_images.pop_back();
        return hip_fail(e, "packet image entry");
    }
    *out = &im;
    return RT_OK;
}

constexpr size_t kMaxConeTabs = 8;
constexpr size_t kConeRingBytes = size_t(16) << 20;

struct TabsWanted {
    bool cone, shadow;
    int shadow_nl;
    bool cls;
    bool clear;
    int cls_kind() const { return cls ? (clear ? 2 : 1) : 0; }
    bool any() const { return cone || shadow; }
};
TabsWanted tables_wanted(const rt_scene* sc, const TraceParams& p) {
    TabsWanted w{false, false, 0, false, false};
    if (!packet_reads_cone_table(p, sc->max_specular > 0.0)) return w;
    const char* e = std::getenv("RTAMD_PK_CONE_TAB");
    w.cone = !(e && std::atoi(e) == 0);
    e = std::getenv("RTAMD_PK_SHADOW_TAB");
    w.shadow = packet_shadow_table_lights(p) > 0 && !(e && std::atoi(e) == 0);
    w.shadow_nl = w.shadow ? packet_shadow_table_lights(p) : 0;
    e = std::getenv("RTAMD_PK_TILE_CLASS");
    w.cls = w.cone && w.shadow && !(e && std::atoi(e) == 0);
    e = std::getenv("RTAMD_PK_PLANE_CLEAR");
    w.clear = w.cls && !(e && std::atoi(e) == 0);
    return w;
}

constexpr size_t kConeKeyWords = rt_scene::PkImage::ConeTab::kKeyWords;
size_t cone_table_key(const TraceParams& p, double dz, int shadow_nl, int cls,
                      uint32_t (&key)[kConeKeyWords], size_t* tiles = nullptr) {
    uint32_t gx, gy, waves;
    packet_grid(p, gx, gy, waves);
    const uint32_t k[9] = {gx, gy, waves, p.width, p.height, p.rows, p.row0, p.row_block,
                           p.row_stride};
    const double c[3] = {dz, p.half_w, p.half_h};
    std::memset(key, 0, sizeof key);
    std::memcpy(key, k, sizeof k);
    std::memcpy(key + 9, c, sizeof c);
    static_assert(sizeof k + sizeof c + 2 * sizeof(uint32_t) + sizeof(double) <=
                      sizeof(uint32_t) * kConeKeyWords, "cone table key");
    if (shadow_nl > 0) {
        key[15] = static_cast<uint32_t>(shadow_nl);
        std::memcpy(key + 16, &p.bias, sizeof p.bias);
        key[18] = cls == 2 ? 3u : (cls ? 1u : 0u);
    }
    const size_t n = static_cast<size_t>(gx) * gy * waves;
    if (tiles) *tiles = n;
    return sizeof(unsigned long long) * n *
           (1 + static_cast<size_t>(shadow_nl > 0 ? shadow_nl + (cls ? 1 : 0) : 0));
}

rt_status cone_table_entry(rt_context* ctx, rt_scene::PkImage& im, const TraceParams& p,
                           double dz, int shadow_nl, int cls,
                           rt_scene::PkImage::ConeTab** tab, bool* fresh) {
    *tab = nullptr;
    *fresh = false;
    uint32_t key[kConeKeyWords];
    const size_t bytes = cone_table_key(p, dz, shadow_nl, cls, key);
    for (auto& t : im.tabs) {
        if (std::memcmp(t.key, key, sizeof key) != 0) continue;
        if (!t.done && t.stream != ctx->stream) {
            const hipError_t q = hipEventQuery(t.ready);
            if (q == hipSuccess) t.done = true;
            else if (q == hipErrorNotReady) RT_HIP(hipStreamWaitEvent(ctx->stream, t.ready, 0));
            else return hip_fail(q, "hipEventQuery");
        }
        *tab = &t;
        return RT_OK;
    }
    if (im.tabs.size() >= kMaxConeTabs) return RT_OK;
    if (im.tabs.capacity() < kMaxConeTabs) im.tabs.reserve(kMaxConeTabs);
    im.tabs.emplace_back();
    auto& t = im.tabs.back();
    std::memcpy(t.key, key, sizeof key);
    t.stream = ctx->stream;
    hipError_t e = t.buf.ensure(bytes);
    if (e == hipSuccess) e = hipEventCreateWithFlags(&t.ready, hipEventDisableTiming);
    if (e != hipSuccess) {
        t.buf.release();
        im.tabs.pop_back();
        return hip_fail(e, "cone table entry");
    }
    *tab = &t;
    *fresh = true;
    return RT_OK;
}

void cone_table_drop(rt_scene::PkImage& im) {
    auto& t = im.tabs.back();
    t.buf.release();
    if (t.ready) (void)hipEventDestroy(t.ready);
    im.tabs.pop_back();
}

rt_status cone_table_single(rt_context* ctx, const rt_scene* sc, rt_scene::PkImage& im,
                            TraceParams& p) {
    const TabsWanted want = tables_wanted(sc, p);
    if (!want.any()) return RT_OK;
    rt_scene::PkImage::ConeTab* t = nullptr;
    bool fresh = false;
    const rt_status st =
        cone_table_entry(ctx, im, p, p.cam_dz, want.shadow_nl, want.cls_kind(), &t, &fresh);
    if (st != RT_OK || !t) return st;
    if (fresh) {
        PkConeJobs jobs;
        std::memset(&jobs, 0, sizeof jobs);
        jobs.dst[0] = static_cast<unsigned long long*>(t->buf.ptr);
        jobs.frame[0] = -1;
        jobs.n = 1;
        jobs.shadow_nl = want.shadow_nl;
        jobs.class_words = want.cls_kind();
        hipError_t e = launch_packet_cone_tables(p, jobs, ctx->stream);
        if (e == hipSuccess) e = hipEventRecord(t->ready, ctx->stream);
        if (e != hipSuccess) {
            cone_table_drop(im);
            return hip_fail(e, "cone table setup");
        }
    }
    uint32_t key[kConeKeyWords];
    size_t tiles = 0;
    (void)cone_table_key(p, p.cam_dz, want.shadow_nl, want.cls_kind(), key, &tiles);
    const unsigned long long* words = static_cast<const unsigned long long*>(t->buf.ptr);
    if (want.cone) p.cone_tab = words;
    if (want.shadow) p.shadow_tab = words + tiles;
    if (want.cls) p.class_tab = words + tiles * (1 + static_cast<size_t>(want.shadow_nl));
    p.plane_masks = want.clear ? 1u : 0u;
    return RT_OK;
}

}

rt_status packet_image(rt_context* ctx, const rt_scene* sc, TraceParams& p, int flags,
                       rt_scene::PkImage::TileOrder** rec) {
    *rec = nullptr;
    rt_scene::PkImage* found = nullptr;
    rt_status st = packet_image_cached(ctx, sc, p.cam_pos, &found);
    if (st != RT_OK) return st;
    if (found) {
        p.pk_image = static_cast<const double*>(found->buf.ptr);
        st = tile_order(ctx, *found, p, flags, rec);
        return st != RT_OK ? st : cone_table_single(ctx, sc, *found, p);
    }
    if (!packet_second_sighting(sc, p.cam_pos)) {
        const rt_status st2 = packet_publish_slot(ctx, sc, p);
        return st2 != RT_OK ? st2 : scene_tile_order(ctx, sc, p, flags, rec);
    }
    rt_scene::PkImage* im = nullptr;
    st = packet_image_entry(ctx, sc, p.cam_pos, p, &im);
    if (st != RT_OK) return st;
    hipError_t e = launch_packet_image(p, static_cast<double*>(im->buf.ptr), ctx->stream);
    if (e == hipSuccess) e = hipEventRecord(im->ready, ctx->stream);
    if (e != hipSuccess) {
        im->buf.release();
        (void)hipEventDestroy(im->ready);
        sc->pk_images.pop_back();
        return hip_fail(e, "packet image setup");
    }
    p.pk_image = static_cast<const double*>(im->buf.ptr);
    st = tile_order(ctx, *im, p, flags, rec);
    return st != RT_OK ? st : cone_table_single(ctx, sc, *im, p);
}

rt_status packet_batch_images(rt_context* ctx, const rt_scene* sc, const rt_camera* cams,
                              int nframes, TraceParams& p, int flags,
                              rt_scene::PkImage::TileOrder** rec, int* batch_ring) {
    *rec = nullptr;
    *batch_ring = -1;
    enum Kind { kCached, kPromote, kRing, kDup };
    Kind kind[kPkMaxBatch];
    int dup_of[kPkMaxBatch];
    rt_scene::PkImage* ent[kPkMaxBatch] = {};
    bool same_cam = true;
    bool any_ring = false;
    const size_t cache_before = sc->pk_images.size();
    struct Rollback {
        const rt_scene* sc;
        size_t keep;
        bool armed = true;
        ~Rollback() {
            if (!armed) return;
            while (sc->pk_images.size() > keep) {
                auto& im = sc->pk_images.back();
                im.buf.release();
                if (im.ready) (void)hipEventDestroy(im.ready);
                sc->pk_images.pop_back();
            }
        }
    } rollback{sc, cache_before};
    for (int f = 0; f < nframes; ++f) {
        PkFrame& F = p.fr[f];
        for (int i = 0; i < 3; ++i) F.cam[i] = cams[f].position[i];
        const CameraConsts cc = camera_consts(p.width, p.height, F.cam[2], p.focal);
        p.fr_dz[f][0] = cc.dz;
        p.fr_dz[f][1] = cc.dz2;
        F.img = nullptr;
        F.pub = nullptr;
        F.epoch = 0;
        F._pad = 0;
        if (std::memcmp(F.cam, p.fr[0].cam, sizeof F.cam) != 0) same_cam = false;
        int g = 0;
        while (g < f && std::memcmp(p.fr[g].cam, F.cam, sizeof F.cam) != 0) ++g;
        if (g < f) {
            kind[f] = kDup;
            dup_of[f] = g;
            continue;
        }
        rt_status st = packet_image_cached(ctx, sc, F.cam, &ent[f]);
        if (st != RT_OK) return st;
        if (ent[f]) {
            kind[f] = kCached;
            F.img = static_cast<const double*>(ent[f]->buf.ptr);
            continue;
        }
        if (packet_second_sighting(sc, F.cam)) {
            st = packet_image_entry(ctx, sc, F.cam, p, &ent[f]);
            if (st != RT_OK) return st;
            kind[f] = kPromote;
            F.img = static_cast<const double*>(ent[f]->buf.ptr);
            continue;
        }
        kind[f] = kRing;
        any_ring = true;
    }
    const size_t img_doubles = ((packet_lds_bytes(p.ns, p.np, p.nl) + 255) & ~size_t(255)) /
                               sizeof(double);
    double* ring = nullptr;
    if (any_ring) {
        const size_t entry = img_doubles * sizeof(double) * kPkMaxBatch;
        RT_HIP(sc->pk_batch.ensure(entry * rt_scene::kPkBatchRing));
        const int r = sc->pk_batch_next;
        sc->pk_batch_next = (r + 1) % rt_scene::kPkBatchRing;
        if (!sc->pk_batch_done[r])
            RT_HIP(hipEventCreateWithFlags(&sc->pk_batch_done[r], hipEventDisableTiming));
        if (sc->pk_batch_used[r])
            RT_HIP(hipStreamWaitEvent(ctx->stream, sc->pk_batch_done[r], 0));
        ring = reinterpret_cast<double*>(static_cast<char*>(sc->pk_batch.ptr) +
                                         static_cast<size_t>(r) * entry);
        *batch_ring = r;
    }
    PkImageJobs jobs;
    std::memset(&jobs, 0, sizeof jobs);
    for (int f = 0; f < nframes; ++f) {
        PkFrame& F = p.fr[f];
        if (kind[f] == kRing) F.img = ring + static_cast<size_t>(f) * img_doubles;
        if (kind[f] == kDup) F.img = p.fr[dup_of[f]].img;
        if (kind[f] == kRing || kind[f] == kPromote) {
            jobs.dst[jobs.n] = const_cast<double*>(F.img);
            jobs.frame[jobs.n] = f;
            ++jobs.n;
        }
    }
    hipError_t e = launch_packet_image_batch(p, jobs, ctx->stream);
    for (int f = 0; f < nframes && e == hipSuccess; ++f)
        if (kind[f] == kPromote) e = hipEventRecord(ent[f]->ready, ctx->stream);
    if (e != hipSuccess) return hip_fail(e, "packet batch images");
    rollback.armed = false;
    const rt_status ost = kind[0] == kCached ? tile_order(ctx, *ent[0], p, flags, rec, !same_cam)
                                             : scene_tile_order(ctx, sc, p, flags, rec);
    const TabsWanted want = tables_wanted(sc, p);
    if (ost != RT_OK || !want.any()) return ost;
    uint32_t key[kConeKeyWords];
    size_t tiles = 0;
    const size_t tab_bytes =
        (cone_table_key(p, 0.0, want.shadow_nl, want.cls_kind(), key, &tiles) + 255) &
        ~size_t(255);
    const size_t cone_bytes =
        (sizeof(unsigned long long) * tiles * (want.cls ? 2 : 1) + 255) & ~size_t(255);
    char* ring_tab = nullptr;
    size_t ring_room = 0;
    if (any_ring) {
        size_t n_ring = 0;
        for (int f = 0; f < nframes; ++f) n_ring += kind[f] == kRing;
        const size_t fit = std::min(n_ring, kConeRingBytes / cone_bytes);
        auto& buf = sc->pk_batch_tab[*batch_ring];
        if (fit > 0 && buf.bytes < fit * tab_bytes) {
            if (sc->pk_batch_used[*batch_ring])
                RT_HIP(hipEventSynchronize(sc->pk_batch_done[*batch_ring]));
            RT_HIP(buf.ensure(fit * tab_bytes));
        }
        ring_tab = static_cast<char*>(buf.ptr);
        ring_room = fit;
    }
    PkConeJobs cj;
    std::memset(&cj, 0, sizeof cj);
    cj.shadow_nl = want.shadow_nl;
    cj.class_words = want.cls_kind();
    p.plane_masks = want.clear ? 1u : 0u;
    auto hand = [&](int f, const unsigned long long* words) {
        p.fr_tab[f] = want.cone ? words : nullptr;
        p.fr_stab[f] = want.shadow ? words + tiles : nullptr;
        p.fr_ctab[f] =
            want.cls ? words + tiles * (1 + static_cast<size_t>(want.shadow_nl)) : nullptr;
    };
    rt_scene::PkImage* made[kPkMaxBatch];
    rt_scene::PkImage::ConeTab* made_tab[kPkMaxBatch];
    int n_made = 0;
    rt_status st = RT_OK;
    for (int f = 0; f < nframes && st == RT_OK; ++f) {
        p.fr_tab[f] = nullptr;
        p.fr_stab[f] = nullptr;
        p.fr_ctab[f] = nullptr;
        unsigned long long* dst = nullptr;
        if (kind[f] == kDup) {
            p.fr_tab[f] = p.fr_tab[dup_of[f]];
            p.fr_stab[f] = p.fr_stab[dup_of[f]];
            p.fr_ctab[f] = p.fr_ctab[dup_of[f]];
            continue;
        }
        if (kind[f] == kRing) {
            if (ring_room == 0) continue;
            --ring_room;
            dst = reinterpret_cast<unsigned long long*>(ring_tab);
            ring_tab += tab_bytes;
        } else {
            rt_scene::PkImage::ConeTab* t = nullptr;
            bool fresh = false;
            st = cone_table_entry(ctx, *ent[f], p, p.fr_dz[f][0], want.shadow_nl,
                                  want.cls_kind(), &t, &fresh);
            if (st != RT_OK || !t) continue;
            hand(f, static_cast<const unsigned long long*>(t->buf.ptr));
            if (!fresh) continue;
            made[n_made] = ent[f];
            made_tab[n_made] = t;
            ++n_made;
            dst = static_cast<unsigned long long*>(t->buf.ptr);
        }
        hand(f, dst);
        cj.dst[cj.n] = dst;
        cj.frame[cj.n] = f;
        ++cj.n;
    }
    if (st == RT_OK) {
        hipError_t ce = launch_packet_cone_tables(p, cj, ctx->stream);
        for (int i = 0; i < n_made && ce == hipSuccess; ++i)
            ce = hipEventRecord(made_tab[i]->ready, ctx->stream);
        if (ce != hipSuccess) st = hip_fail(ce, "packet batch cone tables");
    }
    if (st != RT_OK)
        for (int i = n_made - 1; i >= 0; --i) cone_table_drop(*made[i]);
    return st;
}

}
```

raytracingengine_amd/csrc/rt_packet_kernel.hpp:

```cpp
#pragma once

#include "rt_packet_device.hpp"
#include "rt_shadow_table.hpp"

#pragma clang fp contract(off)

namespace rtamd {

template <int MAXC, int FEAT>
__device__ __forceinline__ double pk_transmittance(const PacketScene& S, const Masks<MAXC>& M,
                                                   int nchunks, d3 o, d3 d, double max_dist,
                                                   double bias) {
    double T = 1.0, traveled = 0.0;
    int safety = 64;
    while (safety-- > 0 && T > 1e-4 && traveled < max_dist) {
        PkHit h;
        if (!closest_masked<MAXC, FEAT>(S, M, nchunks, o, d, h)) break;
        const double t = h.t;
        if (t <= 0.0) {
            o = o + d * bias;
            traveled += bias;
            continue;
        }
        if (t <= bias) {
// ... 237 lines not shown
__device__ __forceinline__ void pk_light_record(const PacketScene& S, const TraceParams& P, int l,
                                                d3& L, d3& E) {
    if constexpr (MAXC == 1) {
        const pk_cdp q = (pk_cdp)P.lt + kLtStride * l;
        L = mk(q[0], q[1], q[2]);
        E = mk(q[3], q[4], q[5]);
    } else {
        const double* q = S.lt + kLtStride * l;
        L = mk(q[0], q[1], q[2]);
        E = mk(q[3], q[4], q[5]);
    }
}

template <int MAXC, int FEAT>
__device__ __forceinline__ d3 pk_uniform_tile(const PacketScene& S, const TraceParams& P,
                                              const double* img, unsigned long long cls, d3 cam,
                                              d3 d, int ns, int np, int nl, double bias,
                                              bool& fix) {
    if (tile_class_of(cls) == kTileSky) return sky(d);
    const int k = static_cast<int>(tile_class_of(cls) - kTilePlane0);
    const pk_cdp pl = (pk_cdp)img + kPkSph * ns;
    const pk_cdp rec = pl + kPlStride * k;
    const pk_cdp on = pl + kPlStride * np + kLtStride * nl + 4 * k;
    const pk_cdp m = (pk_cdp)P.sph_mat + kMatStride * (ns + k);
    const pk_cdp oth = pl + kPlStride * (np > 1 ? 1 - k : k);
    const d3 pp = mk(rec[0], rec[1], rec[2]), pn = mk(rec[3], rec[4], rec[5]);
    const double num = rec[6], core = rec[7];
    const d3 n = mk(on[0], on[1], on[2]);
    bool found = false;
    double t = 0.0;
    int prim = -1;
    const double denom = dot(pn, d);
    if (core != 0.0) plane_t_core(num, denom, ns + k, found, t, prim);
    else plane_t(num, denom, ns + k, found, t, prim);
    const d3 hp = cam + d * t;
    d3 diff = mk(0.0, 0.0, 0.0);
    const d3 spec = mk(0.0, 0.0, 0.0);
    for (int l = 0; l < nl; ++l) {
        d3 lpos, E;
        pk_light_record<MAXC>(S, P, l, lpos, E);
        double dist = 0.0, inv_d2 = 0.0;
        d3 L = mk(0.0, 0.0, 0.0);
        light_dir(lpos - hp, dist, L, inv_d2);
        const bool reach = !(dist <= 0.0);
        if (!reach) L = mk(0.0, 0.0, 0.0);
        const double ndl = smax(0.0, dot(n, L));
        const bool need = reach && !(ndl <= 0.0) && !(dist <= bias);
        const d3 so = hp + n * bias;
        if (!__ballot(need)) continue;
        bool blocked = false, undecided = false;
        const unsigned keep = tile_plane_keep(cls, l);
        if (keep != 0 && need) {
            const double max_dist = dist - bias;
#pragma unroll
            for (int i = 0; i < 2; ++i) {
                if (i >= np) break;
                if (((keep >> (i == 0 ? k : 1 - k)) & 1u) == 0) continue;
                const d3 qp = i == 0 ? pp : mk(oth[0], oth[1], oth[2]);
                const d3 qn = i == 0 ? pn : mk(oth[3], oth[4], oth[5]);
                const double dn = dot(qn, L);
                if (!(fabs(dn) > 1e-6)) continue;
                const double nm = dot(qp - so, qn);
                const double A = dn > 0.0 ? nm : -nm, B = fabs(dn);
                if (A < -1e-300 * B) continue;
                if (A >= max_dist * B * (1.0 + 1e-9)) continue;
                if (A > bias * B * (1.0 + 1e-9) && A < max_dist * B * (1.0 - 1e-9)) blocked = true;
                else undecided = true;
            }
        }
        const double T = (!undecided && blocked) ? 0.0 : 1.0;
        if (undecided) fix = true;
        if (!need) continue;
        if (T <= bias) continue;
        diff = diff + ((E * inv_d2) * ndl) * T;
    }
    const d3 local = hmul(mk(m[0], m[1], m[2]), diff) + spec * m[4];
    const double tr = sclamp(m[5], 0.0, 1.0);
    d3 fin = mk(0.0, 0.0, 0.0);
    if (tr < 1.0) fin = fin + local * (1.0 - tr);
    return fin;
}

constexpr int pk_waves(int MAXC, int FEAT, bool COUNT, bool MULTI) {
    return (FEAT == kFeatFix && MAXC == 1 && !MULTI && !COUNT) ? RT_PACKET_FIX_WAVES
         : (FEAT == 0 && MAXC == 1 && !MULTI && !COUNT) ? RT_PACKET_SMALL_WAVES
         : (FEAT == (kFeatArea | kFeatNoPL) && !MULTI && !COUNT) ? RT_PACKET_AREA_WAVES
         : FEAT == kFeatTris ? RT_PACKET_TRIS_WAVES
         : (((FEAT == 0 || (FEAT & ~kFeatNoPL) == kFeatArea || FEAT == kFeatPlanes) && MAXC <= 4)
                ? (MULTI ? (FEAT == 0 ? RT_PACKET_LEAN_WAVES : 1) : RT_PACKET_AA1_WAVES)
                : 1);
}
template <int MAXC, int FEAT, bool COUNT, bool MULTI, int WGY>
__global__ __launch_bounds__(64 * kWgWavesX * WGY, pk_waves(MAXC, FEAT, COUNT, MULTI)) void packet_direct_kernel(TraceParams P) {
    extern __shared__ __attribute__((aligned(16))) double smem[];
    const int tid = threadIdx.x;
    constexpr bool kNoPL = (FEAT & kFeatNoPL) != 0;
    const uint32_t lin = blockIdx.y * gridDim.x + blockIdx.x;
    uint32_t tbx = blockIdx.x, tby = gridDim.y - 1 - blockIdx.y;
    if (P.tile_order) {
        const uint32_t t = P.tile_order[lin];
        tbx = t % gridDim.x;
        tby = t / gridDim.x;
    }
    uint64_t t_start = 0;
    if constexpr (MULTI)
        if (P.tile_cost) t_start = __builtin_amdgcn_s_memrealtime();
    const int ns = P.ns, np = kNoPL ? 0 : P.np, nl = kNoPL ? 0 : P.nl, nb = pk_chunk_bounds(ns),
              nsb = ns + nb;
    double* s_sph = smem;
    double* s_pl = s_sph + kPkSph * nsb;
    double* s_lt = s_pl + kPlStride * np;
    double* s_pln = s_lt + kLtStride * nl;
    const int32_t* s_orig = reinterpret_cast<const int32_t*>(s_pln + 4 * np);
    const double* camp = P.cam_pos;
    const double* pk_img = P.pk_image;
    unsigned long long* pk_pub = P.pk_pub;
    uint32_t pk_epoch = P.pk_epoch;
    uint64_t frame_off = 0;
    constexpr bool kLean = MAXC == 1 && (FEAT & kFeatArea) == 0;
    constexpr bool kTab = kLean && !MULTI && !COUNT && (FEAT == 0 || FEAT == kFeatFix);
    const unsigned long long* cone_tab = kTab ? P.cone_tab : nullptr;
    const unsigned long long* shadow_tab = kTab ? P.shadow_tab : nullptr;
    constexpr bool kUni = kTab && FEAT == kFeatFix;
    const unsigned long long* class_tab = kUni ? P.class_tab : nullptr;
    double cam_dz = P.cam_dz, cam_dz2 = P.cam_dz2;
    if (P.nframes) {
        const PkFrame& F = P.fr[blockIdx.z];
        camp = F.cam;
        cam_dz = P.fr_dz[blockIdx.z][0];
        cam_dz2 = P.fr_dz[blockIdx.z][1];
        pk_img = F.img;
        pk_pub = F.pub;
        pk_epoch = F.epoch;
        frame_off = static_cast<uint64_t>(blockIdx.z) * P.frame_px;
        if constexpr (kTab) {
            cone_tab = P.fr_tab[blockIdx.z];
            shadow_tab = P.fr_stab[blockIdx.z];
        }
        if constexpr (kUni) class_tab = P.fr_ctab[blockIdx.z];
    }
    const d3 cam = mk(camp[0], camp[1], camp[2]);
    constexpr int kThreads = 64 * kWgWavesX * WGY;
    unsigned long long cls = kTileGeneral;
    bool staged = true;
    if constexpr (kUni) {
        if (class_tab && pk_img && P.max_rec > 0) {
            const pk_culp cw =
                (pk_culp)class_tab + (tby * gridDim.x + tbx) * (kWgWavesX * WGY);
            const uint32_t w = __builtin_amdgcn_readfirstlane(static_cast<uint32_t>(tid >> 6));
            bool all = true;
#pragma unroll
            for (uint32_t i = 0; i < kWgWavesX * WGY; ++i) {
                const unsigned long long c = cw[i];
                all = all && tile_class_of(c) != kTileGeneral;
                if (i == w) cls = c;
            }
            staged = !all;
        }
    }
    if (pk_img && staged) {
        const float4* src = reinterpret_cast<const float4*>(pk_img);
        float4* dst = reinterpret_cast<float4*>(smem);
        const int nv = static_cast<int>(pk_image_bytes(ns, np, nl) / 16);
        for (int i = tid; i < nv; i += kThreads) dst[i] = src[i];
        __syncthreads();
    } else if (pk_img) {
    } else if (pk_pub) {
        uint32_t* dst = reinterpret_cast<uint32_t*>(smem);
        const int nw = static_cast<int>(pk_image_bytes(ns, np, nl) / 4);
        const uint32_t ep = pk_epoch;
        const uint32_t wg = lin;
        bool have = false;
        if (wg >= P.pk_pub_first) {
            int ok = 1;
            for (int i = tid; i < nw / 2; i += kThreads) {
                const unsigned long long gx = __hip_atomic_load(
                    pk_pub + 2 * i, __ATOMIC_RELAXED, __HIP_MEMORY_SCOPE_AGENT);
                const unsigned long long gy = __hip_atomic_load(
                    pk_pub + 2 * i + 1, __ATOMIC_RELAXED, __HIP_MEMORY_SCOPE_AGENT);
                ok &= static_cast<uint32_t>(gx >> 32) == ep && static_cast<uint32_t>(gy >> 32) == ep;
                dst[2 * i] = static_cast<uint32_t>(gx);
                dst[2 * i + 1] = static_cast<uint32_t>(gy);
            }
            have = __syncthreads_and(ok) != 0;
        }
        if (!have) {
            pk_build_image(P, camp, smem, tid, kThreads);
            __syncthreads();
            if (wg == 0) {
                const unsigned long long tag = static_cast<unsigned long long>(ep) << 32;
                for (int i = tid; i < nw; i += kThreads)
                    __hip_atomic_store(pk_pub + i, tag | dst[i], __ATOMIC_RELAXED,
                                       __HIP_MEMORY_SCOPE_AGENT);
            }
        }
    } else {
        pk_build_image(P, camp, smem, tid, kThreads);
        __syncthreads();
    }

    PacketScene S;
    S.sph = s_sph;
    S.pl = s_pl;
    S.lt = s_lt;
    S.tri = P.tri;
    S.mat = P.sph_mat;
    S.bvh = P.bvh;
    S.bvh_tri = P.bvh_tri;
    S.ns = ns;
    S.np = np;
    S.nt = P.nt;
    S.nl = nl;
    S.nb = nb;
    S.orig = nb ? s_orig : nullptr;
    S.wstk = nullptr;
    if constexpr ((FEAT & kFeatTris) != 0)
        S.wstk = reinterpret_cast<int*>(smem + pk_image_bytes(ns, np, nl) / 8) +
                 kPkStack * (tid >> 6);
    const int nchunks = (ns + 63) / 64;

    const int lane = tid & 63, wave = tid >> 6;
    const uint32_t x = tbx * (kPkW * kWgWavesX) + (wave % kWgWavesX) * kPkW + (lane % kPkW);
    const uint32_t yl = tby * (kPkH * WGY) + (wave / kWgWavesX) * kPkH + (lane / kPkW);
    const bool valid = x < P.width && yl < P.rows;
    const uint32_t xc = x < P.width ? x : P.width - 1;
    const uint32_t y = image_row(P, yl < P.rows ? yl : P.rows - 1);
    const uint64_t pix = static_cast<uint64_t>(y) * P.width + xc;
    const double bias = P.bias;
    d3 al_c = mk(0.0, 0.0, 0.0);
    double al_r = 0.0;
    if constexpr ((FEAT & kFeatArea) != 0) {
        const d3 eu = mk(P.al_u[0], P.al_u[1], P.al_u[2]);
        const d3 ev = mk(P.al_v[0], P.al_v[1], P.al_v[2]);
        al_c = (mk(P.al_corner[0], P.al_corner[1], P.al_corner[2]) + eu * 0.5) + ev * 0.5;
        al_r = (0.5 * (length(eu) + length(ev))) * (1.0 + kCullRel);
    }
    Counts cnt{0u, 0u};
    bool fix = false;

    d3 acc = mk(0.0, 0.0, 0.0);
    int samples = 0;
    const int nsamples = MULTI ? P.aa : 1;
    for (int s = 0; s < nsamples; ++s) {
        d3 d;
        if constexpr (kLean) {
            double sx = static_cast<double>(xc) - P.half_w;
            double sy = P.half_h - static_cast<double>(y);
            if constexpr (MULTI) {
                double jx = 0.0, jy = 0.0;
                if (s > 0 && P.aa > 1) {
                    jx = u01(P.seed, pix, static_cast<uint32_t>(s), 0u);
                    jy = u01(P.seed, pix, static_cast<uint32_t>(s), 1u);
                }
                sx += jx;
                sy += jy;
            }
            const d3 dv = mk(sx - cam.x, sy - cam.y, cam_dz);
            d = unit_sq(dv, dv.x * dv.x + dv.y * dv.y + cam_dz2);
        } else {
            d = camera_dir(P, cam, xc, y, pix, s);
        }

        d3 col;
        if (P.max_rec <= 0) {
            col = sky(d);
        } else if (kUni && tile_class_of(cls) != kTileGeneral) {
            if constexpr (kUni)
                col = pk_uniform_tile<MAXC, FEAT>(S, P, pk_img, cls, cam, d, ns, np, nl, bias, fix);
        } else {
            if (COUNT && valid) cnt.trace++;
            const Masks<MAXC> M = [&] {
                if constexpr (kTab) {
                    if (cone_tab) {
                        Masks<MAXC> T;
                        const uint32_t w =
                            __builtin_amdgcn_readfirstlane(static_cast<uint32_t>(wave));
                        T.m[0] = ((pk_culp)cone_tab)[(tby * gridDim.x + tbx) * (kWgWavesX * WGY) + w];
                        T.pm = ~0ull;
                        return T;
                    }
                }
                const d3 axis = lane_d3(d, (kPkH / 2) * kPkW + kPkW / 2);
                const double cos_min =
                    static_cast<double>(wave_red<0>(static_cast<float>(dot(d, axis)))) - 1e-7;
                const bool ok = isfinite(cos_min) && cos_min > 0.0;
                return ok ? cull_cone<MAXC>(S, axis, cos_min) : all_candidates<MAXC>(ns);
            }();
            PkHit h;
            h.t = 0.0;
            h.prim = 0;
            const bool hit = valid && closest_camera<MAXC, FEAT>(S, M, nchunks, cam, d, h);
            const d3 hp = cam + d * h.t;
            d3 view = mk(0.0, 0.0, 0.0);
            d3 inc = mk(0.0, 0.0, 0.0);
            if constexpr ((FEAT & kFeatSpec) != 0) {
                inc = unit(d);
                view = -inc;
            }
            d3 n = mk(0.0, 1.0, 0.0);
            bool known = !hit;
            if (hit && h.prim >= ns && h.prim < ns + np) {
                const double* q = s_pln + 4 * (h.prim - ns);
                if (q[3] != 0.0) {
                    n = mk(q[0], q[1], q[2]);
                    known = true;
                }
            }
            if (!known) {
                const d3 gn = pk_normal(S, h, hp);
                bool front;
                if constexpr ((FEAT & kFeatSpec) != 0) {
                    front = dot(gn, inc) < 0.0;
                } else {
                    const double nd = dot(gn, d);
                    const double sabs = fabs(gn.x * d.x) + fabs(gn.y * d.y) + fabs(gn.z * d.z);
                    if (fabs(nd) > 1e-14 * sabs && sabs > 1e-200) front = nd < 0.0;
                    else front = dot(gn, unit(d)) < 0.0;
                }
                const d3 n0 = front ? gn : -gn;
                n = unit(n0);
            }
            d3 diff = mk(0.0, 0.0, 0.0), spec = mk(0.0, 0.0, 0.0);
            if constexpr (kTab) {
                const unsigned long long* stab = nullptr;
                if (shadow_tab) {
                    const uint32_t w =
                        __builtin_amdgcn_readfirstlane(static_cast<uint32_t>(wave));
                    stab = shadow_tab + static_cast<size_t>(
                               (tby * gridDim.x + tbx) * (kWgWavesX * WGY) + w) * nl;
                }
                for (int l = 0; l < nl; ++l) {
                    d3 L, E;
                    pk_light_record<MAXC>(S, P, l, L, E);
                    pk_light<MAXC, FEAT, COUNT, true>(S, hit, hp, n, view, h, L, E, L, 0.0, bias,
                                                      nchunks, diff, spec, cnt, nullptr, &fix,
                                                      stab ? stab + l : nullptr);
                }
            } else {
                for (int l = 0; l < nl; ++l) {
                    d3 L, E;
                    pk_light_record<MAXC>(S, P, l, L, E);
                    pk_light<MAXC, FEAT, COUNT>(S, hit, hp, n, view, h, L, E, L, 0.0, bias,
                                                nchunks, diff, spec, cnt, nullptr, &fix);
                }
            }
            if constexpr ((FEAT & kFeatArea) != 0) {
                if (P.al_samples > 0) {
                    const uint32_t stream = 0x10000u + (static_cast<uint32_t>(s) << 6);
                    const double k = static_cast<double>(P.al_k);
                    const d3 corner = mk(P.al_corner[0], P.al_corner[1], P.al_corner[2]);
                    const d3 eu = mk(P.al_u[0], P.al_u[1], P.al_u[2]);
                    const d3 ev = mk(P.al_v[0], P.al_v[1], P.al_v[2]);
                    const d3 E = mk(P.al_E[0], P.al_E[1], P.al_E[2]);
                    const OriginBall B = origin_ball(hit, hp + n * bias);
                    const Masks<MAXC> Ma = B.ok ? cull_capsule<MAXC, FEAT>(S, B.c, B.R, al_c, al_r, bias)
                                                : all_candidates<MAXC>(ns);
                    int cand = 0;
#pragma unroll
                    for (int c = 0; c < MAXC; ++c) cand += __builtin_popcountll(Ma.m[c]);
                    const bool per_cell = B.ok && cand > 4;
                    const double cell_r =
                        ((0.5 * (length(eu) + length(ev))) / k) * (1.0 + kCullRel) +
                        1e-12 * (fabs(corner.x) + fabs(corner.y) + fabs(corner.z) + fabs(eu.x) +
                                 fabs(eu.y) + fabs(eu.z) + fabs(ev.x) + fabs(ev.y) + fabs(ev.z));
                    const double rk = rcp_refined(k);
                    for (int q = 0; q < P.al_samples; ++q) {
                        const double r1 = u01(P.seed, pix, stream, 2u * static_cast<uint32_t>(q));
                        const double r2 =
                            u01(P.seed, pix, stream, 2u * static_cast<uint32_t>(q) + 1u);
                        const double fu = div_core(static_cast<double>(q % P.al_k) + r1, k, rk);
                        const double fv = div_core(static_cast<double>(q / P.al_k) + r2, k, rk);
                        const d3 lpos = (corner + eu * fu) + ev * fv;
                        Masks<MAXC> Mq = Ma;
                        if (per_cell) {
                            const double cu = div_core(static_cast<double>(q % P.al_k) + 0.5, k, rk);
                            const double cv = div_core(static_cast<double>(q / P.al_k) + 0.5, k, rk);
                            const Masks<MAXC> Mc = cull_capsule<MAXC, FEAT>(
                                S, B.c, B.R, (corner + eu * cu) + ev * cv, cell_r, bias);
#pragma unroll
                            for (int c = 0; c < MAXC; ++c) Mq.m[c] &= Mc.m[c];
                            Mq.pm &= Mc.pm;
                        }
                        pk_light<MAXC, FEAT, COUNT>(S, hit, hp, n, view, h, lpos, E, al_c, al_r,
                                                    bias, nchunks, diff, spec, cnt, &Mq);
                    }
                }
            }
            if (hit) {
                const double* m = pk_material<MAXC>(S, h);
                const d3 local = hmul(mk(m[0], m[1], m[2]), diff) + spec * m[4];
                const double tr = sclamp(m[5], 0.0, 1.0);
                d3 fin = mk(0.0, 0.0, 0.0);
                if (tr < 1.0) fin = fin + local * (1.0 - tr);
                col = fin;
            } else {
                col = sky(d);
            }
        }
        acc = acc + col;
        samples += 1;
    }
    const uint32_t lane_e = __builtin_amdgcn_mbcnt_hi(~0u, __builtin_amdgcn_mbcnt_lo(~0u, 0u));
    const uint32_t wave_e = __builtin_amdgcn_readfirstlane(static_cast<uint32_t>(wave));
    const uint32_t x_e = tbx * (kPkW * kWgWavesX) + (wave_e % kWgWavesX) * kPkW + (lane_e % kPkW);
    const uint32_t yl_e = tby * (kPkH * WGY) + (wave_e / kWgWavesX) * kPkH + (lane_e / kPkW);
    bool store = x_e < P.width && yl_e < P.rows;
    if constexpr ((FEAT & kFeatFix) != 0) {
        const bool q = fix && store;
        const uint64_t bq = __ballot(q);
        if (bq) {
            uint32_t base = 0;
            if (lane_e == static_cast<uint32_t>(__builtin_ctzll(bq)))
                base = atomicAdd(P.fix_ctl, static_cast<uint32_t>(__builtin_popcountll(bq)));
            base = __shfl(base, __builtin_ctzll(bq), 64);
            if (q)
                P.fix_list[base + __builtin_amdgcn_mbcnt_hi(static_cast<uint32_t>(bq >> 32),
                                                            __builtin_amdgcn_mbcnt_lo(
                                                                static_cast<uint32_t>(bq), 0u))] =
                    static_cast<uint32_t>(frame_off + static_cast<size_t>(yl_e) * P.width + x_e);
        }
        store = store && !fix;
    }
    if (store) {
        const d3 v = samples == 1 ? acc
                   : (samples > 0 ? sdiv(acc, static_cast<double>(samples)) : mk(0.0, 0.0, 0.0));
        const size_t o = frame_off + static_cast<size_t>(yl_e) * P.width + x_e;
        if (P.out64) {
            P.out64[3 * o + 0] = v.x;
            P.out64[3 * o + 1] = v.y;
            P.out64[3 * o + 2] = v.z;
        }
        if (P.out32) {
            P.out32[3 * o + 0] = static_cast<float>(v.x);
            P.out32[3 * o + 1] = static_cast<float>(v.y);
            P.out32[3 * o + 2] = static_cast<float>(v.z);
        }
        if (P.ldr) {
            uint8_t r, g, b;
            if (P.tonemap == 1) {
                r = reinhard_byte(v.x);
                g = reinhard_byte(v.y);
                b = reinhard_byte(v.z);
            } else if constexpr ((FEAT & kFeatJodie) != 0) {
                to_color(tonemap_op(v, P.tonemap), r, g, b);
            } else {
                to_color(tonemap_op_nolog(v, P.tonemap), r, g, b);
            }
            P.ldr[3 * o + 0] = r;
            P.ldr[3 * o + 1] = g;
            P.ldr[3 * o + 2] = b;
        }
    }
    if constexpr (COUNT) {
        uint32_t t = cnt.trace, sh = cnt.shadow;
        for (int off = 32; off > 0; off >>= 1) {
            t += __shfl_xor(t, off, 64);
            sh += __shfl_xor(sh, off, 64);
        }
        if (lane == 0) {
            atomicAdd(P.counters + 0, static_cast<unsigned long long>(t));
            atomicAdd(P.counters + 1, static_cast<unsigned long long>(sh));
        }
    }
    if constexpr (MULTI) {
        if (P.tile_cost && lane == 0 && blockIdx.z == 0) {
            const uint64_t t_end = __builtin_amdgcn_s_memrealtime();
            P.tile_cost[(tby * gridDim.x + tbx) * (kWgWavesX * WGY) + wave] =
                static_cast<uint32_t>(t_end - t_start);
        }
    }
}

template <int MAXC, int FEAT, int WGY>
static void launch_packet_shape(const TraceParams& p, bool count, size_t lds, hipStream_t stream) {
    const dim3 block(64 * kWgWavesX * WGY);
    const dim3 grid((p.width + kPkW * kWgWavesX - 1) / (kPkW * kWgWavesX),
                    (p.rows + kPkH * WGY - 1) / (kPkH * WGY), p.nframes ? p.nframes : 1u);
    if constexpr ((FEAT & kFeatTris) != 0) lds += sizeof(int) * kPkStack * (block.x / 64);
    if (count) hipLaunchKernelGGL((packet_direct_kernel<MAXC, FEAT, true, true, WGY>), grid, block, lds, stream, p);
    else if (p.aa == 1 && !p.tile_cost) hipLaunchKernelGGL((packet_direct_kernel<MAXC, FEAT, false, false, WGY>), grid, block, lds, stream, p);
    else hipLaunchKernelGGL((packet_direct_kernel<MAXC, FEAT, false, true, WGY>), grid, block, lds, stream, p);
}

template <int MAXC, int FEAT>
static void launch_packet_variant(const TraceParams& p, bool count, size_t lds, hipStream_t stream) {
    if (pk_wgy(lds) == 1) launch_packet_shape<MAXC, FEAT, 1>(p, count, lds, stream);
    else launch_packet_shape<MAXC, FEAT, 2>(p, count, lds, stream);
}

hipError_t launch_packet_area(const TraceParams& p, bool count, size_t lds, int chunks,
                              hipStream_t stream);

}
```

raytracingengine_amd/csrc/rt_shadow_table.hpp:

```cpp
#pragma once

#include <math.h>
#include <stdint.h>

#include "rt_cone_table.hpp"

#if defined(__clang__)
#define RT_ST_UNROLL _Pragma("unroll")
#else
#define RT_ST_UNROLL
#endif

namespace rtamd {

constexpr int kShadowTabLights = 4;
constexpr int kShadowTabPlanes = 8;
constexpr unsigned long long kShadowNoWord = ~0ull;
constexpr double kClassMargin = 1e-6;
constexpr unsigned long long kTileGeneral = 0ull, kTileSky = 1ull, kTilePlane0 = 2ull;

RT_CT_HD inline int shadow_table_lights(int ns, int np, int nl, bool area_light) {
    return (!area_light && ns >= 1 && ns <= 63 && np >= 1 && np <= kShadowTabPlanes && nl >= 1 &&
            nl <= kShadowTabLights)
               ? nl
               : 0;
}

struct ShadowBall {
    double c[3];
    float R;
    int plane;
    bool lead;
};
template <int kMaxPlanes = kShadowTabPlanes>
struct ShadowBound {
    ShadowBall ball[kMaxPlanes];
    int n;
    bool ok;
};

template <int kMaxPlanes = kShadowTabPlanes, int kCorners = 4, int kHideCorners = 4,
          bool kBiasInR = true>
RT_CT_HD inline ShadowBound<kMaxPlanes> shadow_tile_bound(const ConeRect& q, double half_w,
                                                          double half_h, const double* cam,
                                                          double dz, const double* planes, int np,
                                                          double bias) {
    ShadowBound<kMaxPlanes> B;
    B.n = 0;
    B.ok = false;
    if (np < 1 || np > kMaxPlanes) return B;
    double v[4][3], vl2_max = 0.0;
    for (int k = 0; k < 4; ++k) {
        v[k][0] = (static_cast<double>((k & 1) ? q.x_hi : q.x_lo) - half_w) - cam[0];
        v[k][1] = (half_h - static_cast<double>((k & 2) ? q.y_hi : q.y_lo)) - cam[1];
        v[k][2] = dz;
        const double l2 = v[k][0] * v[k][0] + v[k][1] * v[k][1] + dz * dz;
        if (!(l2 > 0.0) || !isfinite(l2)) return B;
        if (l2 > vl2_max) vl2_max = l2;
    }
    if (!(dz != 0.0) || !isfinite(dz) || !isfinite(bias)) return B;
    const double cam1 = fabs(cam[0]) + fabs(cam[1]) + fabs(cam[2]);
    if (!isfinite(cam1)) return B;
    double e[kMaxPlanes][4], an[kMaxPlanes];
    bool hit[kMaxPlanes];
    RT_ST_UNROLL
    for (int i = 0; i < kMaxPlanes; ++i) {
        if (i >= np) break;
        const double* p = planes + 8 * i;
        const double num = p[6];
        const double n1 = fabs(p[3]) + fabs(p[4]) + fabs(p[5]);
        if (!(p[7] != 0.0) || !(n1 <= 2.0) || !(n1 >= 0x1p-20) || !(num != 0.0) || !isfinite(num))
            return B;
        if (!(fabs(num) <= 0x1p200) || !(fabs(num) >= 0x1p-200)) return B;
        an[i] = fabs(num);
        int n_hit = 0, n_miss = 0;
        double e_min = INFINITY;
        for (int k = 0; k < 4; ++k) {
            const double a = p[3] * v[k][0], b = p[4] * v[k][1], c = p[5] * v[k][2];
            const double ek = num > 0.0 ? (a + b) + c : -((a + b) + c);
            const double mag = (fabs(a) + fabs(b)) + fabs(c);
            if (!isfinite(ek) || !(fabs(ek) <= 0x1p200)) return B;
            if (ek > 1e-12 * mag) ++n_hit;
            else if (ek <= 0.0) ++n_miss;
            if (fabs(ek) < e_min) e_min = fabs(ek);
            e[i][k] = ek;
// ... 123 lines not shown
        if (b >= B.n) break;
        const ShadowSeg G = shadow_seg(B.ball[b].c, B.ball[b].R, L, bias);
        for (int i = 0; i < ns; ++i)
            if (shadow_seg_keeps(G, B.ball[b].c, sph + static_cast<long>(sph_stride) * i,
                                 rad[static_cast<long>(rad_stride) * i]))
                m |= 1ull << i;
    }
    return m;
}

template <int kMaxPlanes, int kClassPlanes = 1, int kIndexOff = 0>
RT_CT_HD inline unsigned long long tile_class_word(unsigned long long cone,
                                                   const ShadowBound<kMaxPlanes>& B,
                                                   const unsigned long long* words, int nl,
                                                   const double* pln, int np) {
    if (cone != 0 || !B.ok || B.n > kClassPlanes || nl < 1 || nl > kShadowTabLights)
        return kTileGeneral;
    for (int l = 0; l < nl; ++l)
        if (words[l] != 0) return kTileGeneral;
    if (B.n == 0) return kTileSky;
    const int i = B.ball[0].plane;
    if (kClassPlanes == 1 && !B.ball[0].lead) return kTileGeneral;
    if (i < 0 || i >= np || !(pln[4 * i + 3] != 0.0)) return kTileGeneral;
    return kTilePlane0 + static_cast<unsigned long long>((i + kIndexOff) % np);
}

constexpr unsigned kPlaneKeepAll = 0xffu;
template <int kMaxPlanes, bool kSideOfBall = true>
RT_CT_HD inline unsigned shadow_plane_keep(const ShadowBound<kMaxPlanes>& B, const double* L,
                                           const double* planes, int np, const double* cam,
                                           double bias) {
    if (!B.ok || np < 1 || np > kMaxPlanes || np > 8) return kPlaneKeepAll;
    const double ab = fabs(bias);
    const double base = ((fabs(cam[0]) + fabs(cam[1])) + fabs(cam[2])) +
                        ((fabs(L[0]) + fabs(L[1])) + fabs(L[2])) + ab;
    unsigned keep = 0;
    RT_ST_UNROLL
    for (int i = 0; i < kMaxPlanes; ++i) {
        if (i >= np) break;
        const double* p = planes + 8 * i;
        const double N = sqrt((p[3] * p[3] + p[4] * p[4]) + p[5] * p[5]);
        const double p1 = (fabs(p[0]) + fabs(p[1])) + fabs(p[2]);
        const double sL = ((L[0] - p[0]) * p[3] + (L[1] - p[1]) * p[4]) + (L[2] - p[2]) * p[5];
        bool drop = N >= 0x1p-21 && N <= 2.0;
        RT_ST_UNROLL
        for (int b = 0; b < kMaxPlanes; ++b) {
            if (b >= B.n) break;
            const ShadowBall& S = B.ball[b];
            const double R = static_cast<double>(S.R);
            const double scale =
                (base + p1) + (((fabs(S.c[0]) + fabs(S.c[1])) + fabs(S.c[2])) + R);
            if (!(scale >= 0x1p-200 && scale <= 0x1p200)) drop = false;
            if (S.plane == i) {
                if (!(bias >= 1e-7 * scale)) drop = false;
                continue;
            }
            const double m = 1e-6 * scale * N;
            const double sc =
                ((S.c[0] - p[0]) * p[3] + (S.c[1] - p[1]) * p[4]) + (S.c[2] - p[2]) * p[5];
            if (!((sL > 0.0 && sc > 0.0) || (sL < 0.0 && sc < 0.0)) && kSideOfBall) drop = false;
            if (!(fabs(sc) - R * N >= m) && kSideOfBall) drop = false;
            if (!(fabs(sL) - 2.0 * ab * N >= m)) drop = false;
        }
        if (!drop) keep |= 1u << i;
    }
    return keep;
}

constexpr unsigned long long kTileClassBits = 0xffull;
RT_CT_HD inline unsigned long long tile_class_of(unsigned long long word) {
    return word & kTileClassBits;
}
RT_CT_HD inline unsigned long long tile_class_pack(unsigned long long cls, const unsigned* keep,
                                                   int nl) {
    unsigned long long w = cls & kTileClassBits;
    for (int l = 0; l < nl && l < kShadowTabLights; ++l)
        w |= static_cast<unsigned long long>(keep[l] & kPlaneKeepAll) << (8 + 8 * l);
    return w;
}
RT_CT_HD inline unsigned tile_plane_keep(unsigned long long word, int l) {
    return static_cast<unsigned>(word >> (8 + 8 * l)) & kPlaneKeepAll;
}

}
```

Before: 153,400.

## Split packet render into uniform-tile and general-tile kernels via compacted tile lists

The cone-table pass now also compacts tiles into two lists: uniform-class tiles (sky or a single plane) and workgroups that contain any general tile. Tile counts are published to pinned host memory. The renderer then launches a lightweight uniform kernel over the uniform tiles and the general packet kernel only over the listed workgroups, so fully uniform workgroups no longer occupy the heavy kernel. The cost is extra atomics and list writes in the table pass, a host-side read of the counts, and two launches instead of one.

```diff
diff --git a/include/rt_capi.h b/include/rt_capi.h
--- a/include/rt_capi.h
+++ b/include/rt_capi.h
@@ -371,6 +371,8 @@
 
 rt_status rt_debug_plane_clear(rt_context* ctx, uint64_t* with_masks, uint64_t* without_masks);
 
+rt_status rt_debug_tile_split(rt_context* ctx, uint64_t* split, uint64_t* single);
+
 #ifdef __cplusplus
 }
 #endif
diff --git a/raytracingengine_amd/capi.py b/raytracingengine_amd/capi.py
--- a/raytracingengine_amd/capi.py
+++ b/raytracingengine_amd/capi.py
@@ -77,6 +77,7 @@
     "rt_debug_shadow_table",
     "rt_debug_tile_class",
     "rt_debug_plane_clear",
+    "rt_debug_tile_split",
     "rt_occluded_rays", "rt_occluded_rays_device",
     "rt_transmittance_rays", "rt_transmittance_rays_device",
     "rt_light_transmittance", "rt_light_transmittance_device",
@@ -272,6 +273,7 @@
         "rt_debug_shadow_table": [vp, vp, vp],
         "rt_debug_tile_class": [vp, vp, vp],
         "rt_debug_plane_clear": [vp, vp, vp],
+        "rt_debug_tile_split": [vp, vp, vp],
         "rt_debug_assemble_rows": [vp, vp, ctypes.c_size_t, ctypes.c_uint32, ctypes.c_uint32,
                                    ctypes.c_uint32, ctypes.c_uint32, vp],
     }.items():
@@ -418,6 +420,11 @@
     def debug_plane_clear(self) -> tuple[int, int]:
         a, b = ctypes.c_uint64(), ctypes.c_uint64()
         _check(_lib.rt_debug_plane_clear(self._h, ctypes.byref(a), ctypes.byref(b)))
+        return a.value, b.value
+
+    def debug_tile_split(self) -> tuple[int, int]:
+        a, b = ctypes.c_uint64(), ctypes.c_uint64()
+        _check(_lib.rt_debug_tile_split(self._h, ctypes.byref(a), ctypes.byref(b)))
         return a.value, b.value
 
     def debug_vec_ops(self, v: np.ndarray) -> np.ndarray:
diff --git a/raytracingengine_amd/csrc/rt_capi.cpp b/raytracingengine_amd/csrc/rt_capi.cpp
--- a/raytracingengine_amd/csrc/rt_capi.cpp
+++ b/raytracingengine_amd/csrc/rt_capi.cpp
@@ -308,10 +308,11 @@
     const bool packet = packet_path;
     rt_scene::PkImage::TileOrder* rec = nullptr;
     int batch_ring = -1;
+    PkSplit pk_split{0u, 0u, 0u};
     if (packet && nframes > 1) {
         p.nframes = static_cast<uint32_t>(nframes);
         p.frame_px = frame_px;
-        st = packet_batch_images(ctx, sc, cams, nframes, p, flags, &rec, &batch_ring);
+        st = packet_batch_images(ctx, sc, cams, nframes, p, flags, &rec, &batch_ring, &pk_split);
         if (st != RT_OK) return st;
     } else if (packet) {
         st = packet_image(ctx, sc, p, flags, &rec);
@@ -343,6 +344,9 @@
         st = scratch_wait(ctx);
         if (st != RT_OK) return st;
     }
+    if (!fixup || p.tile_order) pk_split.tiles = 0;
+    if (packet && fixup)
+        (pk_split.tiles ? ctx->tile_split_frames : ctx->tile_nosplit_frames) += nframes;
     const bool lean_generic = p.nt == 0 && p.al_samples == 0;
     static const bool box_sph = [] {
         const char* e = std::getenv("RTAMD_BOX_SPH");
@@ -355,7 +359,8 @@
     auto launch = [&](const TraceParams& q, bool count) {
         if (box)
             return launch_box_chain(q, count, !(flags & RT_FLAG_NO_SAMPLE_PARALLEL), ctx->stream);
-        return packet ? launch_packet_direct(q, count, sc->max_specular > 0.0, ctx->stream)
+        return packet ? launch_packet_direct(q, count, sc->max_specular > 0.0, ctx->stream,
+                                             count ? nullptr : &pk_split)
                       : (lean_generic ? lean::launch_trace(q, path, count, lds, lds_bytes, ctx->stream, spar)
                                       : launch_trace(q, path, count, lds, lds_bytes, ctx->stream, spar));
     };
@@ -764,6 +769,7 @@
         for (auto& t : im.tabs) {
             t.buf.release();
             if (t.ready) (void)hipEventDestroy(t.ready);
+            if (t.counts) (void)hipHostFree(t.counts);
         }
     }
     for (auto& b : sc->pk_batch_tab) b.release();
@@ -1793,6 +1799,14 @@
     return RT_OK;
 }
 
+rt_status rt_debug_tile_split(rt_context* ctx, uint64_t* split, uint64_t* single) {
+    if (!ctx || !split || !single)
+        return fail(RT_ERR_INVALID_ARG, "NULL argument to rt_debug_tile_split");
+    *split = ctx->tile_split_frames;
+    *single = ctx->tile_nosplit_frames;
+    return RT_OK;
+}
+
 rt_status rt_debug_vec_ops(rt_context* ctx, const double* v, size_t n, double* out) {
     if (!ctx || !v || !out) return fail(RT_ERR_INVALID_ARG, "NULL argument");
     DeviceGuard g(ctx->device);
diff --git a/raytracingengine_amd/csrc/rt_context.hpp b/raytracingengine_amd/csrc/rt_context.hpp
--- a/raytracingengine_amd/csrc/rt_context.hpp
+++ b/raytracingengine_amd/csrc/rt_context.hpp
@@ -76,6 +76,7 @@
     uint64_t shadow_tab_frames = 0, shadow_notab_frames = 0;
     uint64_t tile_class_frames = 0, tile_noclass_frames = 0;
     uint64_t plane_mask_frames = 0, plane_nomask_frames = 0;
+    uint64_t tile_split_frames = 0, tile_nosplit_frames = 0;
     std::vector<rt_context*> group_ctxs;
     std::vector<rt_comm*> group_comms;
     std::vector<rt_context*> group_roots;
@@ -118,6 +119,7 @@
             hipEvent_t ready = nullptr;
             hipStream_t stream = nullptr;
             bool done = false;
+            unsigned long long* counts = nullptr;
         };
         std::vector<ConeTab> tabs;
     };
@@ -146,7 +148,8 @@
                        rt_scene::PkImage::TileOrder** rec);
 rt_status packet_batch_images(rt_context* ctx, const rt_scene* sc, const rt_camera* cams,
                               int nframes, TraceParams& p, int flags,
-                              rt_scene::PkImage::TileOrder** rec, int* batch_ring);
+                              rt_scene::PkImage::TileOrder** rec, int* batch_ring,
+                              PkSplit* split);
 bool uses_wavefront_arena(int path, int flags);
 rt_status scratch_wait(rt_context* ctx);
 rt_status scratch_done(rt_context* ctx);
diff --git a/raytracingengine_amd/csrc/rt_internal.hpp b/raytracingengine_amd/csrc/rt_internal.hpp
--- a/raytracingengine_amd/csrc/rt_internal.hpp
+++ b/raytracingengine_amd/csrc/rt_internal.hpp
@@ -98,6 +98,10 @@
     const unsigned long long* class_tab;
     const unsigned long long* fr_ctab[kPkMaxBatch];
 };
+struct PkSplit {
+    uint32_t tiles;
+    uint32_t uni_n, gen_n;
+};
 static_assert(sizeof(TraceParams) + 12 * kPkMaxBatch + 32 <= 4096, "kernel arguments above 4 KiB");
 
 struct CameraConsts {
@@ -134,7 +138,7 @@
 hipError_t launch_box_chain(const TraceParams& p, bool count, bool sample_parallel,
                             hipStream_t stream);
 hipError_t launch_packet_direct(const TraceParams& p, bool count, bool any_specular,
-                                hipStream_t stream);
+                                hipStream_t stream, const PkSplit* split = nullptr);
 size_t packet_lds_bytes(int ns, int np, int nl);
 hipError_t launch_packet_image(const TraceParams& p, double* img, hipStream_t stream);
 bool packet_uses_fixup(const TraceParams& p, bool count, bool any_specular);
@@ -152,9 +156,14 @@
     int32_t n;
     int32_t shadow_nl;
     int32_t class_words;
+    int32_t lists;
+};
+struct PkListCounts {
+    unsigned long long* host[kPkMaxBatch];
 };
 hipError_t launch_packet_cone_tables(const TraceParams& p, const PkConeJobs& jobs,
-                                     hipStream_t stream);
+                                     hipStream_t stream, const PkListCounts* counts = nullptr);
+bool packet_split_wanted(const TraceParams& p);
 bool packet_reads_cone_table(const TraceParams& p, bool any_specular);
 int packet_shadow_table_lights(const TraceParams& p);
 void packet_grid(const TraceParams& p, uint32_t& gx, uint32_t& gy, uint32_t& waves);
diff --git a/raytracingengine_amd/csrc/rt_packet.hip b/raytracingengine_amd/csrc/rt_packet.hip
--- a/raytracingengine_amd/csrc/rt_packet.hip
+++ b/raytracingengine_amd/csrc/rt_packet.hip
@@ -55,8 +55,9 @@
         for (int i = threadIdx.x; i < 3 * ns; i += kConeThreads)
             s_ctr[i] = img[kPkSph * (i / 3) + i % 3];
     __syncthreads();
-    const uint32_t t = blockIdx.x * kConeThreads + threadIdx.x;
-    if (t >= gx * gy * waves) return;
+    const uint32_t pos = blockIdx.x * kConeThreads + threadIdx.x;
+    if (pos >= gx * gy * waves) return;
+    const uint32_t t = J.lists ? tile_list_tile(pos, gx * gy * waves) : pos;
     const uint32_t wave = t % waves, wg = t / waves, tbx = wg % gx, tby = wg / gx;
     const uint32_t x0 = tbx * (kPkW * kWgWavesX) + (wave % kWgWavesX) * kPkW;
     const uint32_t yl0 = tby * (kPkH * (waves / kWgWavesX)) + (wave / kWgWavesX) * kPkH;
@@ -85,12 +86,46 @@
     }
     if (J.class_words == 0) return;
     const double* pln = img + kPkSph * ns + kPlStride * P.np + kLtStride * P.nl;
-    J.dst[blockIdx.y][static_cast<size_t>(gx) * gy * waves * (1 + J.shadow_nl) + t] =
-        tile_class_word(cone, SB, &any, 1, pln, P.np) | keep;
+    const unsigned long long cw = tile_class_word(cone, SB, &any, 1, pln, P.np) | keep;
+    J.dst[blockIdx.y][static_cast<size_t>(gx) * gy * waves * (1 + J.shadow_nl) + t] = cw;
+    if (!J.lists) return;
+    const size_t tiles = static_cast<size_t>(gx) * gy * waves;
+    unsigned long long* hdr = J.dst[blockIdx.y] + tiles * (2 + J.shadow_nl);
+    unsigned long long* uni = hdr + 1;
+    uint32_t* gen = reinterpret_cast<uint32_t*>(hdr + 1 + tiles);
+    const uint32_t lane = threadIdx.x & 63u;
+    const bool is_uni = tile_list_uniform(cw);
+    const uint64_t bu = __ballot(is_uni), bg = __ballot(!is_uni);
+    const bool lead = (lane & (waves - 1u)) == 0 && tile_list_wg_listed(bg, lane, waves);
+    const uint64_t bl = __ballot(lead);
+    uint32_t base_u = 0, base_g = 0;
+    if (lane == 0) {
+        if (bu) base_u = atomicAdd(reinterpret_cast<uint32_t*>(hdr),
+                                   static_cast<uint32_t>(__builtin_popcountll(bu)));
+        if (bl) base_g = atomicAdd(reinterpret_cast<uint32_t*>(hdr) + 1,
+                                   static_cast<uint32_t>(__builtin_popcountll(bl)));
+    }
+    base_u = __shfl(base_u, 0, 64);
+    base_g = __shfl(base_g, 0, 64);
+    const uint64_t below = (1ull << lane) - 1ull;
+    if (is_uni) uni[base_u + __builtin_popcountll(bu & below)] = tile_list_entry(cw, x0, yl0);
+    if (lead) gen[base_g + __builtin_popcountll(bl & below)] = wg;
+}
+
+__global__ __launch_bounds__(64) void packet_list_zero_kernel(PkConeJobs J, size_t hdr) {
+    if (static_cast<int>(threadIdx.x) < J.n) J.dst[threadIdx.x][hdr] = 0ull;
+}
+__global__ __launch_bounds__(64) void packet_list_counts_kernel(PkConeJobs J, PkListCounts C,
+                                                                size_t hdr) {
+    if (static_cast<int>(threadIdx.x) >= J.n || !C.host[threadIdx.x]) return;
+    const unsigned long long v = J.dst[threadIdx.x][hdr];
+    __hip_atomic_store(C.host[threadIdx.x],
+                       (((v >> 32) + 1ull) << 32) | ((v & 0xffffffffull) + 1ull), __ATOMIC_RELAXED,
+                       __HIP_MEMORY_SCOPE_SYSTEM);
 }
 
 hipError_t launch_packet_cone_tables(const TraceParams& p, const PkConeJobs& jobs,
-                                     hipStream_t stream) {
+                                     hipStream_t stream, const PkListCounts* counts) {
     if (jobs.n <= 0) return hipSuccess;
     if (jobs.n > kPkMaxBatch || p.ns > 64 || p.width == 0 || p.rows == 0)
         return hipErrorInvalidValue;
@@ -98,6 +133,7 @@
         return hipErrorInvalidValue;
     if (jobs.class_words != 0 && jobs.shadow_nl <= 0) return hipErrorInvalidValue;
     if (jobs.class_words < 0 || jobs.class_words > 2) return hipErrorInvalidValue;
+    if (jobs.lists != 0 && jobs.class_words == 0) return hipErrorInvalidValue;
     for (int j = 0; j < jobs.n; ++j) {
         const int f = jobs.frame[j];
         if (!jobs.dst[j] || f < -1 || f >= static_cast<int>(p.nframes) ||
@@ -107,10 +143,19 @@
     uint32_t gx, gy, waves;
     packet_grid(p, gx, gy, waves);
     const uint32_t tiles = gx * gy * waves;
+    const size_t hdr = static_cast<size_t>(tiles) * (2 + jobs.shadow_nl);
+    if (jobs.lists) {
+        if (gx * kWgWavesX > kListMaxCoord || gy * (waves / kWgWavesX) > kListMaxCoord)
+            return hipErrorInvalidValue;
+        hipLaunchKernelGGL(packet_list_zero_kernel, dim3(1), dim3(64), 0, stream, jobs, hdr);
+    }
     hipLaunchKernelGGL(packet_cone_table_kernel,
                        dim3((tiles + kConeThreads - 1) / kConeThreads,
                             static_cast<unsigned>(jobs.n)),
                        dim3(kConeThreads), 0, stream, p, jobs, gx, gy, waves);
+    if (jobs.lists && counts)
+        hipLaunchKernelGGL(packet_list_counts_kernel, dim3(1), dim3(64), 0, stream, jobs, *counts,
+                           hdr);
     return hipGetLastError();
 }
 
@@ -285,14 +330,86 @@
     return eligible && (mode == 1 || px >= kPkFixMinPixels);
 }
 
+#ifndef RT_PACKET_UNI_THREADS
+#define RT_PACKET_UNI_THREADS 256
+#endif
+#ifndef RT_PACKET_UNI_WAVES
+#define RT_PACKET_UNI_WAVES 8
+#endif
+constexpr int kUniThreads = RT_PACKET_UNI_THREADS;
+__global__ __launch_bounds__(kUniThreads, RT_PACKET_UNI_WAVES) void packet_uniform_kernel(TraceParams P, uint32_t tiles) {
+    constexpr int FEAT = kFeatFix;
+    const PkFrame& F = P.fr[blockIdx.z];
+    const pk_culp hdr = (pk_culp)P.fr_ctab[blockIdx.z] + tiles;
+    const uint32_t i = blockIdx.x * (kUniThreads / 64) +
+                       __builtin_amdgcn_readfirstlane(static_cast<uint32_t>(threadIdx.x) >> 6);
+    if (i >= static_cast<uint32_t>(hdr[0])) return;
+    const unsigned long long e = hdr[1 + i];
+    const unsigned long long cls = e & kListWordMask;
+    const uint32_t col = static_cast<uint32_t>(e >> kListColShift) & kListCoordMask;
+    const uint32_t row = static_cast<uint32_t>(e >> kListRowShift) & kListCoordMask;
+    const d3 cam = mk(F.cam[0], F.cam[1], F.cam[2]);
+    const double cam_dz = P.fr_dz[blockIdx.z][0], cam_dz2 = P.fr_dz[blockIdx.z][1];
+    const uint64_t frame_off = static_cast<uint64_t>(blockIdx.z) * P.frame_px;
+    const uint32_t lane = __builtin_amdgcn_mbcnt_hi(~0u, __builtin_amdgcn_mbcnt_lo(~0u, 0u));
+    const uint32_t x = col * kPkW + (lane % kPkW), yl = row * kPkH + (lane / kPkW);
+    const uint32_t xc = x < P.width ? x : P.width - 1;
+    const uint32_t y = image_row(P, yl < P.rows ? yl : P.rows - 1);
+    const double sx = static_cast<double>(xc) - P.half_w;
+    const double sy = P.half_h - static_cast<double>(y);
+    const d3 dv = mk(sx - cam.x, sy - cam.y, cam_dz);
+    const d3 d = unit_sq(dv, dv.x * dv.x + dv.y * dv.y + cam_dz2);
+    bool fix = false;
+    PacketScene S;
+    S.lt = nullptr;
+    const d3 col3 = pk_uniform_tile<1, FEAT>(S, P, F.img, cls, cam, d, P.ns, P.np, P.nl, P.bias, fix);
+    const d3 acc = mk(0.0, 0.0, 0.0) + col3;
+    constexpr int samples = 1;
+    const uint32_t lane_e = lane, x_e = x, yl_e = yl;
+#include "rt_packet_epilogue.hpp"
+}
+
+bool packet_split_wanted(const TraceParams& p) {
+    const char* e = std::getenv("RTAMD_PK_TILE_SPLIT");
+    if (e && std::atoi(e) == 0) return false;
+    uint32_t gx, gy, waves;
+    packet_grid(p, gx, gy, waves);
+    return !p.tile_order && waves == kWgWavesX && gx * kWgWavesX <= kListMaxCoord &&
+           gy <= kListMaxCoord;
+}
+
+static void launch_packet_split(const TraceParams& p, const PkSplit& s, size_t lds,
+                                hipStream_t stream) {
+    const dim3 block(64 * kWgWavesX);
+    const dim3 ggrid(s.gen_n, 1u, p.nframes);
+    const dim3 ugrid((s.uni_n + kUniThreads / 64 - 1) / (kUniThreads / 64), 1u, p.nframes);
+#ifdef RT_PACKET_SPLIT_GENERAL_FIRST
+    if (s.gen_n)
+        hipLaunchKernelGGL((packet_direct_kernel<1, kFeatFix | kFeatSplit, false, false, 1>),
+                           ggrid, block, lds, stream, p);
+#endif
+    if (s.uni_n)
+        hipLaunchKernelGGL(packet_uniform_kernel, ugrid, dim3(kUniThreads), 0, stream, p,
+                           s.tiles);
+#ifndef RT_PACKET_SPLIT_GENERAL_FIRST
+    if (s.gen_n)
+        hipLaunchKernelGGL((packet_direct_kernel<1, kFeatFix | kFeatSplit, false, false, 1>),
+                           ggrid, block, lds, stream, p);
+#endif
+}
+
 hipError_t launch_packet_direct(const TraceParams& p, bool count, bool any_specular,
-                                hipStream_t stream) {
+                                hipStream_t stream, const PkSplit* split) {
     const size_t lds = packet_lds_bytes(p.ns, p.np, p.nl);
     const int chunks = (p.ns + 63) / 64;
     int feat = packet_features(p, any_specular);
     if (packet_uses_fixup(p, count, any_specular)) {
         if (!p.fix_list || !p.fix_ctl || !p.fix_next) return hipErrorInvalidValue;
         feat = kFeatFix;
+        if (split && split->tiles) {
+            launch_packet_split(p, *split, lds, stream);
+            return hipGetLastError();
+        }
     }
     if (feat == kFeatArea) return launch_packet_area(p, count, lds, chunks, stream);
     if (chunks <= 1) launch_packet_maxc<1>(p, count, lds, feat, stream);
diff --git a/raytracingengine_amd/csrc/rt_packet_device.hpp b/raytracingengine_amd/csrc/rt_packet_device.hpp
--- a/raytracingengine_amd/csrc/rt_packet_device.hpp
+++ b/raytracingengine_amd/csrc/rt_packet_device.hpp
@@ -38,6 +38,10 @@
 constexpr int kFeatFix = 128;
 #ifndef RT_PACKET_FIX_WAVES
 #define RT_PACKET_FIX_WAVES 8
+#endif
+constexpr int kFeatSplit = 256;
+#ifndef RT_PACKET_GENERAL_WAVES
+#define RT_PACKET_GENERAL_WAVES RT_PACKET_FIX_WAVES
 #endif
 
 constexpr int kPkStack = 64;
diff --git a/raytracingengine_amd/csrc/rt_packet_epilogue.hpp b/raytracingengine_amd/csrc/rt_packet_epilogue.hpp
--- /dev/null
+++ b/raytracingengine_amd/csrc/rt_packet_epilogue.hpp
@@ -0,0 +1,47 @@
+    bool store = x_e < P.width && yl_e < P.rows;
+    if constexpr ((FEAT & kFeatFix) != 0) {
+        const bool q = fix && store;
+        const uint64_t bq = __ballot(q);
+        if (bq) {
+            uint32_t base = 0;
+            if (lane_e == static_cast<uint32_t>(__builtin_ctzll(bq)))
+                base = atomicAdd(P.fix_ctl, static_cast<uint32_t>(__builtin_popcountll(bq)));
+            base = __shfl(base, __builtin_ctzll(bq), 64);
+            if (q)
+                P.fix_list[base + __builtin_amdgcn_mbcnt_hi(static_cast<uint32_t>(bq >> 32),
+                                                            __builtin_amdgcn_mbcnt_lo(
+                                                                static_cast<uint32_t>(bq), 0u))] =
+                    static_cast<uint32_t>(frame_off + static_cast<size_t>(yl_e) * P.width + x_e);
+        }
+        store = store && !fix;
+    }
+    if (store) {
+        const d3 v = samples == 1 ? acc
+                   : (samples > 0 ? sdiv(acc, static_cast<double>(samples)) : mk(0.0, 0.0, 0.0));
+        const size_t o = frame_off + static_cast<size_t>(yl_e) * P.width + x_e;
+        if (P.out64) {
+            P.out64[3 * o + 0] = v.x;
+            P.out64[3 * o + 1] = v.y;
+            P.out64[3 * o + 2] = v.z;
+        }
+        if (P.out32) {
+            P.out32[3 * o + 0] = static_cast<float>(v.x);
+            P.out32[3 * o + 1] = static_cast<float>(v.y);
+            P.out32[3 * o + 2] = static_cast<float>(v.z);
+        }
+        if (P.ldr) {
+            uint8_t r, g, b;
+            if (P.tonemap == 1) {
+                r = reinhard_byte(v.x);
+                g = reinhard_byte(v.y);
+                b = reinhard_byte(v.z);
+            } else if constexpr ((FEAT & kFeatJodie) != 0) {
+                to_color(tonemap_op(v, P.tonemap), r, g, b);
+            } else {
+                to_color(tonemap_op_nolog(v, P.tonemap), r, g, b);
+            }
+            P.ldr[3 * o + 0] = r;
+            P.ldr[3 * o + 1] = g;
+            P.ldr[3 * o + 2] = b;
+        }
+    }
diff --git a/raytracingengine_amd/csrc/rt_packet_host.cpp b/raytracingengine_amd/csrc/rt_packet_host.cpp
--- a/raytracingengine_amd/csrc/rt_packet_host.cpp
+++ b/raytracingengine_amd/csrc/rt_packet_host.cpp
@@ -8,6 +8,7 @@
 
 #include "rt_context.hpp"
 #include "rt_internal.hpp"
+#include "rt_shadow_table.hpp"
 
 #pragma clang fp contract(off)
 
@@ -171,11 +172,12 @@
     int shadow_nl;
     bool cls;
     bool clear;
+    bool lists;
     int cls_kind() const { return cls ? (clear ? 2 : 1) : 0; }
     bool any() const { return cone || shadow; }
 };
 TabsWanted tables_wanted(const rt_scene* sc, const TraceParams& p) {
-    TabsWanted w{false, false, 0, false, false};
+    TabsWanted w{false, false, 0, false, false, false};
     if (!packet_reads_cone_table(p, sc->max_specular > 0.0)) return w;
     const char* e = std::getenv("RTAMD_PK_CONE_TAB");
     w.cone = !(e && std::atoi(e) == 0);
@@ -186,11 +188,13 @@
     w.cls = w.cone && w.shadow && !(e && std::atoi(e) == 0);
     e = std::getenv("RTAMD_PK_PLANE_CLEAR");
     w.clear = w.cls && !(e && std::atoi(e) == 0);
+    w.lists = w.cls && p.nframes >= 1 && packet_uses_fixup(p, false, sc->max_specular > 0.0) &&
+              packet_split_wanted(p);
     return w;
 }
 
 constexpr size_t kConeKeyWords = rt_scene::PkImage::ConeTab::kKeyWords;
-size_t cone_table_key(const TraceParams& p, double dz, int shadow_nl, int cls,
+size_t cone_table_key(const TraceParams& p, double dz, int shadow_nl, int cls, bool lists,
                       uint32_t (&key)[kConeKeyWords], size_t* tiles = nullptr) {
     uint32_t gx, gy, waves;
     packet_grid(p, gx, gy, waves);
@@ -205,21 +209,22 @@
     if (shadow_nl > 0) {
         key[15] = static_cast<uint32_t>(shadow_nl);
         std::memcpy(key + 16, &p.bias, sizeof p.bias);
-        key[18] = cls == 2 ? 3u : (cls ? 1u : 0u);
+        key[18] = (cls == 2 ? 3u : (cls ? 1u : 0u)) | (cls && lists ? 4u : 0u);
     }
     const size_t n = static_cast<size_t>(gx) * gy * waves;
     if (tiles) *tiles = n;
-    return sizeof(unsigned long long) * n *
-           (1 + static_cast<size_t>(shadow_nl > 0 ? shadow_nl + (cls ? 1 : 0) : 0));
+    return sizeof(unsigned long long) *
+           (n * (1 + static_cast<size_t>(shadow_nl > 0 ? shadow_nl + (cls ? 1 : 0) : 0)) +
+            (shadow_nl > 0 && cls && lists ? tile_list_words(n, static_cast<size_t>(gx) * gy) : 0));
 }
 
 rt_status cone_table_entry(rt_context* ctx, rt_scene::PkImage& im, const TraceParams& p,
-                           double dz, int shadow_nl, int cls,
+                           double dz, int shadow_nl, int cls, bool lists,
                            rt_scene::PkImage::ConeTab** tab, bool* fresh) {
     *tab = nullptr;
     *fresh = false;
     uint32_t key[kConeKeyWords];
-    const size_t bytes = cone_table_key(p, dz, shadow_nl, cls, key);
+    const size_t bytes = cone_table_key(p, dz, shadow_nl, cls, lists, key);
     for (auto& t : im.tabs) {
         if (std::memcmp(t.key, key, sizeof key) != 0) continue;
         if (!t.done && t.stream != ctx->stream) {
@@ -239,8 +244,13 @@
     t.stream = ctx->stream;
     hipError_t e = t.buf.ensure(bytes);
     if (e == hipSuccess) e = hipEventCreateWithFlags(&t.ready, hipEventDisableTiming);
+    if (e == hipSuccess && lists) {
+        e = hipHostMalloc(reinterpret_cast<void**>(&t.counts), sizeof(unsigned long long));
+        if (e == hipSuccess) __atomic_store_n(t.counts, 0ull, __ATOMIC_RELAXED);
+    }
     if (e != hipSuccess) {
         t.buf.release();
+        if (t.ready) (void)hipEventDestroy(t.ready);
         im.tabs.pop_back();
         return hip_fail(e, "cone table entry");
     }
@@ -253,6 +263,7 @@
     auto& t = im.tabs.back();
     t.buf.release();
     if (t.ready) (void)hipEventDestroy(t.ready);
+    if (t.counts) (void)hipHostFree(t.counts);
     im.tabs.pop_back();
 }
 
@@ -262,8 +273,8 @@
     if (!want.any()) return RT_OK;
     rt_scene::PkImage::ConeTab* t = nullptr;
     bool fresh = false;
-    const rt_status st =
-        cone_table_entry(ctx, im, p, p.cam_dz, want.shadow_nl, want.cls_kind(), &t, &fresh);
+    const rt_status st = cone_table_entry(ctx, im, p, p.cam_dz, want.shadow_nl, want.cls_kind(),
+                                          false, &t, &fresh);
     if (st != RT_OK || !t) return st;
     if (fresh) {
         PkConeJobs jobs;
@@ -282,7 +293,7 @@
     }
     uint32_t key[kConeKeyWords];
     size_t tiles = 0;
-    (void)cone_table_key(p, p.cam_dz, want.shadow_nl, want.cls_kind(), key, &tiles);
+    (void)cone_table_key(p, p.cam_dz, want.shadow_nl, want.cls_kind(), false, key, &tiles);
     const unsigned long long* words = static_cast<const unsigned long long*>(t->buf.ptr);
     if (want.cone) p.cone_tab = words;
     if (want.shadow) p.shadow_tab = words + tiles;
@@ -326,9 +337,11 @@
 
 rt_status packet_batch_images(rt_context* ctx, const rt_scene* sc, const rt_camera* cams,
                               int nframes, TraceParams& p, int flags,
-                              rt_scene::PkImage::TileOrder** rec, int* batch_ring) {
+                              rt_scene::PkImage::TileOrder** rec, int* batch_ring,
+                              PkSplit* split) {
     *rec = nullptr;
     *batch_ring = -1;
+    *split = PkSplit{0u, 0u, 0u};
     enum Kind { kCached, kPromote, kRing, kDup };
     Kind kind[kPkMaxBatch];
     int dup_of[kPkMaxBatch];
@@ -420,12 +433,13 @@
     rollback.armed = false;
     const rt_status ost = kind[0] == kCached ? tile_order(ctx, *ent[0], p, flags, rec, !same_cam)
                                              : scene_tile_order(ctx, sc, p, flags, rec);
-    const TabsWanted want = tables_wanted(sc, p);
+    TabsWanted want = tables_wanted(sc, p);
     if (ost != RT_OK || !want.any()) return ost;
+    if (any_ring) want.lists = false;
     uint32_t key[kConeKeyWords];
     size_t tiles = 0;
     const size_t tab_bytes =
-        (cone_table_key(p, 0.0, want.shadow_nl, want.cls_kind(), key, &tiles) + 255) &
+        (cone_table_key(p, 0.0, want.shadow_nl, want.cls_kind(), want.lists, key, &tiles) + 255) &
         ~size_t(255);
     const size_t cone_bytes =
         (sizeof(unsigned long long) * tiles * (want.cls ? 2 : 1) + 255) & ~size_t(255);
@@ -448,6 +462,20 @@
     std::memset(&cj, 0, sizeof cj);
     cj.shadow_nl = want.shadow_nl;
     cj.class_words = want.cls_kind();
+    cj.lists = want.lists ? 1 : 0;
+    PkListCounts lc;
+    std::memset(&lc, 0, sizeof lc);
+    uint32_t gx, gy, waves;
+    packet_grid(p, gx, gy, waves);
+    uint32_t n_uni = 0, n_gen = 0;
+    bool all_lists = want.lists;
+    auto count_frame = [&](const unsigned long long* host) {
+        const unsigned long long v = host ? __atomic_load_n(host, __ATOMIC_RELAXED) : 0ull;
+        const uint32_t u = static_cast<uint32_t>(v), g = static_cast<uint32_t>(v >> 32);
+        if (!u || !g) all_lists = false;
+        n_uni = std::max(n_uni, u ? u - 1u : static_cast<uint32_t>(tiles));
+        n_gen = std::max(n_gen, g ? g - 1u : gx * gy);
+    };
     p.plane_masks = want.clear ? 1u : 0u;
     auto hand = [&](int f, const unsigned long long* words) {
         p.fr_tab[f] = want.cone ? words : nullptr;
@@ -471,6 +499,7 @@
             continue;
         }
         if (kind[f] == kRing) {
+            if (ring_room == 0) all_lists = false;
             if (ring_room == 0) continue;
             --ring_room;
             dst = reinterpret_cast<unsigned long long*>(ring_tab);
@@ -479,28 +508,35 @@
             rt_scene::PkImage::ConeTab* t = nullptr;
             bool fresh = false;
             st = cone_table_entry(ctx, *ent[f], p, p.fr_dz[f][0], want.shadow_nl,
-                                  want.cls_kind(), &t, &fresh);
+                                  want.cls_kind(), want.lists, &t, &fresh);
+            if (st != RT_OK || !t) all_lists = false;
             if (st != RT_OK || !t) continue;
             hand(f, static_cast<const unsigned long long*>(t->buf.ptr));
+            if (!fresh) count_frame(t->counts);
             if (!fresh) continue;
+            lc.host[cj.n] = t->counts;
             made[n_made] = ent[f];
             made_tab[n_made] = t;
             ++n_made;
             dst = static_cast<unsigned long long*>(t->buf.ptr);
         }
         hand(f, dst);
+        count_frame(nullptr);
         cj.dst[cj.n] = dst;
         cj.frame[cj.n] = f;
         ++cj.n;
     }
     if (st == RT_OK) {
-        hipError_t ce = launch_packet_cone_tables(p, cj, ctx->stream);
+        hipError_t ce = launch_packet_cone_tables(p, cj, ctx->stream, &lc);
         for (int i = 0; i < n_made && ce == hipSuccess; ++i)
             ce = hipEventRecord(made_tab[i]->ready, ctx->stream);
         if (ce != hipSuccess) st = hip_fail(ce, "packet batch cone tables");
     }
     if (st != RT_OK)
         for (int i = n_made - 1; i >= 0; --i) cone_table_drop(*made[i]);
+    if (st == RT_OK && all_lists) {
+        *split = PkSplit{static_cast<uint32_t>(tiles), n_uni, n_gen};
+    }
     return st;
 }
 
diff --git a/raytracingengine_amd/csrc/rt_packet_kernel.hpp b/raytracingengine_amd/csrc/rt_packet_kernel.hpp
--- a/raytracingengine_amd/csrc/rt_packet_kernel.hpp
+++ b/raytracingengine_amd/csrc/rt_packet_kernel.hpp
@@ -343,7 +343,9 @@
 }
 
 constexpr int pk_waves(int MAXC, int FEAT, bool COUNT, bool MULTI) {
-    return (FEAT == kFeatFix && MAXC == 1 && !MULTI && !COUNT) ? RT_PACKET_FIX_WAVES
+    return (FEAT == (kFeatFix | kFeatSplit) && MAXC == 1 && !MULTI && !COUNT)
+               ? RT_PACKET_GENERAL_WAVES
+         : (FEAT == kFeatFix && MAXC == 1 && !MULTI && !COUNT) ? RT_PACKET_FIX_WAVES
          : (FEAT == 0 && MAXC == 1 && !MULTI && !COUNT) ? RT_PACKET_SMALL_WAVES
          : (FEAT == (kFeatArea | kFeatNoPL) && !MULTI && !COUNT) ? RT_PACKET_AREA_WAVES
          : FEAT == kFeatTris ? RT_PACKET_TRIS_WAVES
@@ -351,17 +353,22 @@
                 ? (MULTI ? (FEAT == 0 ? RT_PACKET_LEAN_WAVES : 1) : RT_PACKET_AA1_WAVES)
                 : 1);
 }
-template <int MAXC, int FEAT, bool COUNT, bool MULTI, int WGY>
-__global__ __launch_bounds__(64 * kWgWavesX * WGY, pk_waves(MAXC, FEAT, COUNT, MULTI)) void packet_direct_kernel(TraceParams P) {
+template <int MAXC, int FEAT_, bool COUNT, bool MULTI, int WGY>
+__global__ __launch_bounds__(64 * kWgWavesX * WGY, pk_waves(MAXC, FEAT_, COUNT, MULTI)) void packet_direct_kernel(TraceParams P) {
+    constexpr int FEAT = FEAT_ & ~kFeatSplit;
+    constexpr bool SPLIT = (FEAT_ & kFeatSplit) != 0;
     extern __shared__ __attribute__((aligned(16))) double smem[];
     const int tid = threadIdx.x;
     constexpr bool kNoPL = (FEAT & kFeatNoPL) != 0;
     const uint32_t lin = blockIdx.y * gridDim.x + blockIdx.x;
     uint32_t tbx = blockIdx.x, tby = gridDim.y - 1 - blockIdx.y;
-    if (P.tile_order) {
-        const uint32_t t = P.tile_order[lin];
-        tbx = t % gridDim.x;
-        tby = t / gridDim.x;
+    const uint32_t gxw = SPLIT ? (P.width + kPkW * kWgWavesX - 1) / (kPkW * kWgWavesX) : gridDim.x;
+    if constexpr (!SPLIT) {
+        if (P.tile_order) {
+            const uint32_t t = P.tile_order[lin];
+            tbx = t % gridDim.x;
+            tby = t / gridDim.x;
+        }
     }
     uint64_t t_start = 0;
     if constexpr (MULTI)
@@ -382,8 +389,8 @@
     constexpr bool kTab = kLean && !MULTI && !COUNT && (FEAT == 0 || FEAT == kFeatFix);
     const unsigned long long* cone_tab = kTab ? P.cone_tab : nullptr;
     const unsigned long long* shadow_tab = kTab ? P.shadow_tab : nullptr;
-    constexpr bool kUni = kTab && FEAT == kFeatFix;
-    const unsigned long long* class_tab = kUni ? P.class_tab : nullptr;
+    constexpr bool kUni = kTab && FEAT == kFeatFix && !SPLIT;
+    const unsigned long long* class_tab = (kUni || SPLIT) ? P.class_tab : nullptr;
     double cam_dz = P.cam_dz, cam_dz2 = P.cam_dz2;
     if (P.nframes) {
         const PkFrame& F = P.fr[blockIdx.z];
@@ -398,7 +405,16 @@
             cone_tab = P.fr_tab[blockIdx.z];
             shadow_tab = P.fr_stab[blockIdx.z];
         }
-        if constexpr (kUni) class_tab = P.fr_ctab[blockIdx.z];
+        if constexpr (kUni || SPLIT) class_tab = P.fr_ctab[blockIdx.z];
+    }
+    if constexpr (SPLIT) {
+        const uint32_t split_tiles =
+            gxw * ((P.rows + kPkH * WGY - 1) / (kPkH * WGY)) * (kWgWavesX * WGY);
+        const pk_culp hdr = (pk_culp)class_tab + split_tiles;
+        if (lin >= static_cast<uint32_t>(hdr[0] >> 32)) return;
+        const uint32_t t = ((pk_cip)(hdr + 1 + split_tiles))[lin];
+        tbx = t % gxw;
+        tby = t / gxw;
     }
     const d3 cam = mk(camp[0], camp[1], camp[2]);
     constexpr int kThreads = 64 * kWgWavesX * WGY;
@@ -407,7 +423,7 @@
     if constexpr (kUni) {
         if (class_tab && pk_img && P.max_rec > 0) {
             const pk_culp cw =
-                (pk_culp)class_tab + (tby * gridDim.x + tbx) * (kWgWavesX * WGY);
+                (pk_culp)class_tab + (tby * gxw + tbx) * (kWgWavesX * WGY);
             const uint32_t w = __builtin_amdgcn_readfirstlane(static_cast<uint32_t>(tid >> 6));
             bool all = true;
 #pragma unroll
@@ -418,6 +434,10 @@
             }
             staged = !all;
         }
+    }
+    if constexpr (SPLIT) {
+        const uint32_t w = __builtin_amdgcn_readfirstlane(static_cast<uint32_t>(tid >> 6));
+        cls = ((pk_culp)class_tab)[(tby * gxw + tbx) * (kWgWavesX * WGY) + w];
     }
     if (pk_img && staged) {
         const float4* src = reinterpret_cast<const float4*>(pk_img);
@@ -425,6 +445,8 @@
         const int nv = static_cast<int>(pk_image_bytes(ns, np, nl) / 16);
         for (int i = tid; i < nv; i += kThreads) dst[i] = src[i];
         __syncthreads();
+        if constexpr (SPLIT)
+            if (tile_class_of(cls) != kTileGeneral) return;
     } else if (pk_img) {
     } else if (pk_pub) {
         uint32_t* dst = reinterpret_cast<uint32_t*>(smem);
@@ -536,7 +558,7 @@
                         Masks<MAXC> T;
                         const uint32_t w =
                             __builtin_amdgcn_readfirstlane(static_cast<uint32_t>(wave));
-                        T.m[0] = ((pk_culp)cone_tab)[(tby * gridDim.x + tbx) * (kWgWavesX * WGY) + w];
+                        T.m[0] = ((pk_culp)cone_tab)[(tby * gxw + tbx) * (kWgWavesX * WGY) + w];
                         T.pm = ~0ull;
                         return T;
                     }
@@ -588,7 +610,7 @@
                     const uint32_t w =
                         __builtin_amdgcn_readfirstlane(static_cast<uint32_t>(wave));
                     stab = shadow_tab + static_cast<size_t>(
-                               (tby * gridDim.x + tbx) * (kWgWavesX * WGY) + w) * nl;
+                               (tby * gxw + tbx) * (kWgWavesX * WGY) + w) * nl;
                 }
                 for (int l = 0; l < nl; ++l) {
                     d3 L, E;
@@ -665,53 +687,7 @@
     const uint32_t wave_e = __builtin_amdgcn_readfirstlane(static_cast<uint32_t>(wave));
     const uint32_t x_e = tbx * (kPkW * kWgWavesX) + (wave_e % kWgWavesX) * kPkW + (lane_e % kPkW);
     const uint32_t yl_e = tby * (kPkH * WGY) + (wave_e / kWgWavesX) * kPkH + (lane_e / kPkW);
-    bool store = x_e < P.width && yl_e < P.rows;
-    if constexpr ((FEAT & kFeatFix) != 0) {
-        const bool q = fix && store;
-        const uint64_t bq = __ballot(q);
-        if (bq) {
-            uint32_t base = 0;
-            if (lane_e == static_cast<uint32_t>(__builtin_ctzll(bq)))
-                base = atomicAdd(P.fix_ctl, static_cast<uint32_t>(__builtin_popcountll(bq)));
-            base = __shfl(base, __builtin_ctzll(bq), 64);
-            if (q)
-                P.fix_list[base + __builtin_amdgcn_mbcnt_hi(static_cast<uint32_t>(bq >> 32),
-                                                            __builtin_amdgcn_mbcnt_lo(
-                                                                static_cast<uint32_t>(bq), 0u))] =
-                    static_cast<uint32_t>(frame_off + static_cast<size_t>(yl_e) * P.width + x_e);
-        }
-        store = store && !fix;
-    }
-    if (store) {
-        const d3 v = samples == 1 ? acc
-                   : (samples > 0 ? sdiv(acc, static_cast<double>(samples)) : mk(0.0, 0.0, 0.0));
-        const size_t o = frame_off + static_cast<size_t>(yl_e) * P.width + x_e;
-        if (P.out64) {
-            P.out64[3 * o + 0] = v.x;
-            P.out64[3 * o + 1] = v.y;
-            P.out64[3 * o + 2] = v.z;
-        }
-        if (P.out32) {
-            P.out32[3 * o + 0] = static_cast<float>(v.x);
-            P.out32[3 * o + 1] = static_cast<float>(v.y);
-            P.out32[3 * o + 2] = static_cast<float>(v.z);
-        }
-        if (P.ldr) {
-            uint8_t r, g, b;
-            if (P.tonemap == 1) {
-                r = reinhard_byte(v.x);
-                g = reinhard_byte(v.y);
-                b = reinhard_byte(v.z);
-            } else if constexpr ((FEAT & kFeatJodie) != 0) {
-                to_color(tonemap_op(v, P.tonemap), r, g, b);
-            } else {
-                to_color(tonemap_op_nolog(v, P.tonemap), r, g, b);
-            }
-            P.ldr[3 * o + 0] = r;
-            P.ldr[3 * o + 1] = g;
-            P.ldr[3 * o + 2] = b;
-        }
-    }
+#include "rt_packet_epilogue.hpp"
     if constexpr (COUNT) {
         uint32_t t = cnt.trace, sh = cnt.shadow;
         for (int off = 32; off > 0; off >>= 1) {
diff --git a/raytracingengine_amd/csrc/rt_shadow_table.hpp b/raytracingengine_amd/csrc/rt_shadow_table.hpp
--- a/raytracingengine_amd/csrc/rt_shadow_table.hpp
+++ b/raytracingengine_amd/csrc/rt_shadow_table.hpp
@@ -1,6 +1,7 @@
 #pragma once
 
 #include <math.h>
+#include <stddef.h>
 #include <stdint.h>
 
 #include "rt_cone_table.hpp"
@@ -290,4 +291,47 @@
     return static_cast<unsigned>(word >> (8 + 8 * l)) & kPlaneKeepAll;
 }
 
-}
+constexpr int kListColShift = 40, kListRowShift = 52;
+constexpr unsigned long long kListWordMask = (1ull << kListColShift) - 1ull;
+constexpr uint32_t kListCoordMask = 0xfffu;
+constexpr uint32_t kListMaxCoord = kListCoordMask + 1u;
+RT_CT_HD inline size_t tile_list_words(size_t tiles, size_t wgs) {
+    return 1 + tiles + (wgs + 1) / 2;
+}
+RT_CT_HD inline uint32_t tile_list_tile(uint32_t pos, uint32_t tiles) { return tiles - 1u - pos; }
+RT_CT_HD inline bool tile_list_uniform(unsigned long long word) {
+    return tile_class_of(word) != kTileGeneral;
+}
+template <int kIndexOff = 0>
+RT_CT_HD inline unsigned long long tile_list_entry(unsigned long long word, uint32_t x0,
+                                                   uint32_t yl0) {
+    return (word & kListWordMask) |
+           (static_cast<unsigned long long>((x0 / 8u + kIndexOff) & kListCoordMask) << kListColShift) |
+           (static_cast<unsigned long long>((yl0 / 8u) & kListCoordMask) << kListRowShift);
+}
+template <bool kDropMixed = false>
+RT_CT_HD inline bool tile_list_wg_listed(uint64_t general, unsigned lane, unsigned waves) {
+    const uint64_t group = (waves >= 64u ? ~0ull : (1ull << waves) - 1ull);
+    const uint64_t g = (general >> (lane & ~(waves - 1u))) & group;
+    return kDropMixed ? g == group : g != 0;
+}
+template <int kIndexOff = 0, bool kDropMixed = false, class Origin>
+inline void tile_list_run(const unsigned long long* words, uint32_t tiles, uint32_t waves,
+                          uint32_t pos0, Origin origin, unsigned long long* uni, uint32_t* n_uni,
+                          uint32_t* gen, uint32_t* n_gen) {
+    uint64_t general = 0;
+    for (uint32_t l = 0; l < 64 && pos0 + l < tiles; ++l)
+        if (!tile_list_uniform(words[tile_list_tile(pos0 + l, tiles)])) general |= 1ull << l;
+    for (uint32_t l = 0; l < 64 && pos0 + l < tiles; ++l) {
+        const uint32_t t = tile_list_tile(pos0 + l, tiles);
+        if (tile_list_uniform(words[t])) {
+            uint32_t x0, yl0;
+            origin(t, x0, yl0);
+            uni[(*n_uni)++] = tile_list_entry<kIndexOff>(words[t], x0, yl0);
+        }
+        if ((l & (waves - 1u)) == 0 && tile_list_wg_listed<kDropMixed>(general, l, waves))
+            gen[(*n_gen)++] = t / waves;
+    }
+}
+
+}
```

Result: faster. 164,600 (median of 6 runs) (+7.3%).
